# johndpope/SPEAK-hack

Measured on AMD Instinct MI355X. Metric: generator frames/sec at 256^2, batch 8/GPU, higher is better.
Workload: dtype f32; 1 GPU; StyleGAN decoder (styleganv1.StyleGenerator) 256^2 forward only, batch 8/GPU, fp32, random-init weights, synthetic [8,6144] latents, device-drawn noise; global_batch=8, resolution=256, parallelism=replicas x1 (no data-path collective), launch=hipGraph replay of the step

## Files before the change

include/spk.h:

```cpp
#ifndef SPK_H_
#define SPK_H_

#include <stddef.h>
#include <stdint.h>

#ifdef __cplusplus
extern "C" {
#endif

#define SPK_OK            0
#define SPK_EINVAL       -1
#define SPK_ELAUNCH      -2
#define SPK_EUNSUPPORTED -3

#define SPK_EPI_BIAS   1u
#define SPK_EPI_NOISE  2u
#define SPK_EPI_LRELU  4u
#define SPK_EPI_STYLE  8u
#define SPK_CONV_UPSAMPLE2X 16u
#define SPK_EPI_ACCUM  32u
#define SPK_EPI_STATS  64u
#define SPK_CONV_IN_AFFINE_RELU 128u
#define SPK_CONV_IN_BATCH_SCALE 256u
#define SPK_CONV_DGRAD_S2 1024u
#define SPK_CONV_TRANSPOSE4X4_S2 2048u
#define SPK_CONV_BF16X3 4096u
#define SPK_CONV_WINOGRAD 16384u
#define SPK_EPI_ACCUM_HALF 8192u
#define SPK_EPI_TORGB 32768u
#define SPK_EPI_RESIDUAL 65536u
#define SPK_CONV_UP_FIR1331 512u

const char* spk_version(void);
const char* spk_last_error(void);

typedef struct spk_conv2d_desc {
    const float* x;
    const float* w_packed;
    const float* bias;
    const float* noise_w;
    const float* noise;
    const float* style;
    const float* in_scale;
    const float* in_shift;
    double*      stats;
    float*       y;
    float*       y_pre;
    int32_t B, Cin, Cout;
    int32_t H, W;
    int32_t Hin, Win;
    int32_t kh, kw, stride;
    int32_t style_stride;
    uint32_t flags;
    float lrelu_slope;
    float out_scale;
    int32_t config;
    int32_t ksplit;
    void*   workspace;
    int64_t workspace_bytes;
    const float* out_scale_bc;
    float act_gain;
    int32_t groups;
    int32_t group_in_stride;
    int32_t stats_slots;
    const float* accum_half;
    const float* out_scale_dev;
    const float* rgb_w;
    const float* rgb_bias;
    float* rgb_y;
    int32_t rgb_channels;
    int32_t reserved;
    const float* residual;
} spk_conv2d_desc;

int spk_conv2d_num_configs(void);
int spk_conv2d_stats_slots(int config, int kh, int kw, int stride, int B, int Cin, int Cout, int H, int W);
int spk_conv2d_config_valid(int config, int kh, int kw, int stride);
int spk_conv2d_pick_config(int kh, int kw, int stride, int B, int Cin, int Cout, int H, int W);
int spk_conv2d_dgrad_s2_config(int B, int Cin, int Cout, int Hin, int Win);
int64_t spk_conv2d_dgrad_s2_workspace_bytes(int B, int Cin, int Cout, int Hin, int Win, int H, int W, int groups);
int spk_conv2d_config_info(int config, int* co_tile, int* ci_tile, int* pix_tile);
int64_t spk_conv2d_packed_floats(int config, int kh, int kw, int Cin, int Cout);
int64_t spk_conv2d_workspace_bytes(int config, int ksplit, int kh, int kw, int stride, int B, int Cin, int Cout,
                                   int H, int W);
int64_t spk_conv2d_workspace_bytes_grouped(int config, int ksplit, int kh, int kw, int stride, int B, int Cin, int Cout,
                                           int H, int W, int groups);
int spk_conv2d_pack_weights(const float* w, float* w_packed, int kh, int kw, int Cin, int Cout, int config,
                            int transpose_flip, void* stream);
#define SPK_PACK_LIST_MAX 8
int spk_conv2d_pack_weights_list(const float* const* ws, int n, float* w_packed, int kh, int kw, int Cin, int Cout, int config,
                                 int transpose_flip, void* stream);
int spk_conv2d_fwd(const spk_conv2d_desc* desc, void* stream);
int64_t spk_conv2d_packed_bytes_bf16x3(int Cin, int Cout);
int spk_conv2d_pack_weights_bf16x3(const float* w, void* w_packed, int Cin, int Cout, void* stream);
int spk_conv2d_pack_weights_bf16x3_tf(const float* w, void* w_packed, int Cin, int Cout, int transpose_flip, void* stream);
int spk_conv2d_bf16x3_supported(int B, int Cin, int Cout, int H, int W);
int spk_conv2d_bf16x3_fwd(const spk_conv2d_desc* desc, void* stream);

int64_t spk_conv2d_packed_bytes_wino(int Cin, int Cout);
int spk_conv2d_pack_weights_wino(const float* w, float* w_packed, int Cin, int Cout, int transpose_flip, void* stream);
#define SPK_WINO_PACK_MAX 32
int spk_conv2d_pack_weights_wino_list(const float* const* w, float* const* w_packed, const int* Cin, const int* Cout, const int* transpose_flip,
                                      int n, void* stream);
int spk_conv2d_wino_supported(int B, int Cin, int Cout, int H, int W);
int spk_conv2d_wino_up_supported(int B, int Cin, int Cout, int H, int W);
int spk_conv2d_wino_ksplit(int want, int B, int Cin, int Cout, int H, int W);
int64_t spk_conv2d_wino_workspace_bytes(int ksplit, int B, int Cin, int Cout, int H, int W);
int spk_conv2d_wino_fwd(const spk_conv2d_desc* desc, void* stream);

typedef struct spk_wgrad_desc {
    const float* g;
    const float* x;
    const float* in_scale;
    const float* in_shift;
    float*       dw;
    int32_t B, Cin, Cout, H, W, Hin, Win, kh, kw, stride;
    uint32_t flags;
    float scale;
    int32_t accumulate;
    int32_t splits;
    void*   workspace;
    int64_t workspace_bytes;
    int32_t groups;
    int32_t group_in_stride;
    int32_t fold;
    const float* g_scale;
} spk_wgrad_desc;
int64_t spk_conv2d_wgrad_workspace_bytes(int kh, int kw, int stride, int splits, int B, int Cin, int Cout, int H, int W);
int spk_conv2d_wgrad(const spk_wgrad_desc* desc, void* stream);
int spk_conv2d_wgrad_up_supported(int B, int Cin, int Cout, int H, int W);
int spk_conv2d_wgrad_mod_supported(int B, int Cin, int Cout, int H, int W, int upsample);
int spk_conv2d_wgrad_wino_supported(int B, int Cin, int Cout, int H, int W);
int spk_conv2d_wgrad_wino_splits(int splits, int B, int Cin, int Cout, int H, int W);
int64_t spk_conv2d_wgrad_wino_workspace_bytes(int splits, int B, int Cin, int Cout, int H, int W);
int spk_conv2d_wgrad_wino(const spk_wgrad_desc* desc, void* stream);
int spk_wgrad_reduce_slabs(const float* slabs, float* dw, int n_slabs, int Cout, int Cin, int taps, float scale, int accumulate, int fold,
                           void* stream);

int spk_epilogue_bwd(const float* dy, const float* a, const float* noise, const float* style, int64_t style_stride,
                     float slope, float* dt, float* sums, int B, int C, int64_t HW, void* stream);
int spk_upsample2x_bilinear_bwd(const float* dy, float* dx, int64_t planes, int Hin, int Win, void* stream);
int spk_conv1x1_small_bwd_blocks(int B, int64_t HW);
int spk_conv1x1_small_bwd(const float* x, const float* w, const float* dy, float* dx, float* partial, int B, int C, int O,
                          int64_t HW, float in_scale, void* stream);
int spk_fc_bwd(const float* dout, const float* out, const float* x, int64_t x_stride, const float* w, float* dx,
               int64_t dx_stride, float* dw, float* db, int B, int I, int O, float wmul, float bmul, float slope,
               void* stream);

int spk_fc_fwd(const float* x, int64_t x_stride, const float* w, const float* bias, float* out,
               int64_t out_stride, int B, int I, int O, float wmul, float bmul, float slope, void* stream);

#define SPK_FC_MAX_GROUPS 16
typedef struct spk_fc_group {
    const float* x;
    int64_t x_stride;
    const float* w;
    const float* bias;
    float* out;
    int64_t out_stride;
    int32_t I, O;
    float wmul, bmul, slope;
    int32_t reserved;
} spk_fc_group;
int spk_fc_grouped_fwd(const spk_fc_group* groups, int n_groups, int B, void* stream);
typedef struct spk_fc_bwd_group {
    const float* dout;
    int64_t dout_stride;
    const float* out;
    const float* x;
    int64_t x_stride;
    const float* w;
    float* dx;
    int64_t dx_stride;
    float* dw;
    float* db;
    int32_t I, O;
    float wmul, bmul, slope;
    int32_t reserved;
} spk_fc_bwd_group;
int spk_fc_grouped_bwd(const spk_fc_bwd_group* groups, int n_groups, int B, void* stream);

int spk_bias_noise_style_fwd(const float* x, int64_t x_batch_stride, const float* bias, const float* noise_w,
                             const float* noise, const float* style, int64_t style_stride, float* y, int B, int C,
                             int HW, void* stream);

int spk_conv1x1_expand_fwd(const float* x, const float* w, const float* bias, const float* scale_dev, float* y, int B, int C, int O,
                           int64_t HW, float slope, void* stream);
int spk_conv1x1_small_fwd(const float* x, const float* w, const float* bias, float* y, int B, int C, int O,
                          int64_t HW, float in_scale, void* stream);

int spk_upsample2x_bilinear_fwd(const float* x, float* y, int64_t planes, int Hin, int Win, void* stream);
int spk_upsample2x_fwd(const float* x, float* y, int64_t planes, int Hin, int Win, int zero_border, void* stream);

int spk_bn_finalize(double* stats, int stats_slots, int64_t count, const float* gamma, const float* beta, float* running_mean,
                    float* running_var, float momentum, float eps, float* scale, float* shift, float* save_mean,
                    float* save_invstd, int C, void* stream);
#define SPK_BN_LIST_MAX 64
typedef struct spk_bn_replay_item {
    const double* stats;
    float* running_mean;
    float* running_var;
    int64_t count;
    int32_t C;
    int32_t reserved;
} spk_bn_replay_item;
int spk_bn_replay_list(const spk_bn_replay_item* items_host, int n, float momentum, void* stream);
int spk_bn_add_relu_fwd(const float* a, const float* sa, const float* ba, const float* b, const float* sb,
                        const float* bb, float* y, int B, int C, int64_t HW, int relu, void* stream);
int spk_maxpool3x3s2_fwd(const float* x, const float* in_scale, const float* in_shift, float* y, int B, int C,
                         int Hin, int Win, void* stream);
int spk_bn_bwd_reduce(const float* g, const float* r, const float* mask_src, int mask_mode, const float* scale,
                      const float* shift, const float* mean, const float* invstd, float g_scale, int g_per_plane,
                      float* sums, int B, int C, int64_t HW, void* stream);
int spk_bn_bwd_apply(const float* g, const float* r, const float* mask_src, int mask_mode, const float* scale,
                     const float* shift, const float* mean, const float* invstd, const float* csum, int64_t count,
                     float g_scale, int g_per_plane, float* dr, float* dz_out, int B, int C, int64_t HW, void* stream);
int spk_bn_bwd_apply_sums(const float* g, const float* r, const float* mask_src, int mask_mode, const float* scale,
                          const float* shift, const float* mean, const float* invstd, const float* sums, float* csum_out,
                          int batch_stats, int64_t count, float g_scale, int g_per_plane, float* dr, float* dz_out, int B, int C,
                          int64_t HW, void* stream);
int spk_dilate2x(const float* x, float* y, int64_t planes, int H, int W, int Ho, int Wo, void* stream);
int spk_maxpool3x3s2_bwd(const float* x, const float* in_scale, const float* in_shift, const float* dy, float* dx, int B,
                         int C, int Hin, int Win, void* stream);
int spk_global_avgpool_fwd(const float* x, float* y, int64_t planes, int64_t HW, void* stream);

int spk_modconv_demod(const float* w, const float* s, float* d, int B, int Cin, int Cout, int taps, float scale, float eps,
                      void* stream);
int spk_modconv_epi_finish(const float* sums, const float* d, const float* bias, const float* noise_w, float gain, float* dd,
                           float* dprime, float* dbias, float* dnw, int B, int C, void* stream);
int spk_modconv_dx_finish(const float* dxt, const float* x, const float* s, float* dx, float* ds, int B, int C, int Hs, int Ws,
                          int upsample, void* stream);
int64_t spk_modconv_demod_bwd_workspace_bytes(int B, int Cin, int Cout);
int spk_modconv_demod_bwd(const float* w, const float* s, const float* d, const float* dd, float* ds, float* dw, void* workspace,
                          int64_t workspace_bytes, int B, int Cin, int Cout, int taps, float scale, void* stream);
int spk_torgb_mod_bwd_data(const float* w, const float* mod, const float* dy, float* dx, int B, int C, int O, int64_t HW,
                           float in_scale, void* stream);
#define SPK_DEMOD_MAX_GROUPS 16
typedef struct spk_demod_group {
    const float* w;
    const float* s;
    float* d;
    int32_t Cin, Cout, taps;
    float scale;
} spk_demod_group;
int spk_modconv_demod_grouped(const spk_demod_group* groups, int n_groups, int B, float eps, void* stream);
int spk_upfirdn2d_fwd(const float* x, float* y, const float* filter_host, int k, int64_t planes, int H, int W, int up, int down,
                      int pad0, int pad1, float gain, void* stream);
int spk_conv1x1_small_mod_fwd(const float* x, const float* w, const float* mod, const float* bias, float* y, int B, int C, int O,
                              int64_t HW, float in_scale, void* stream);
int spk_torgb_mod_skip_fwd(const float* x, const float* w, const float* mod, const float* bias, const float* skip, float* y, int B,
                           int C, int O, int H, int W, float in_scale, void* stream);

int spk_pixelnorm_fwd(const float* x, float* y, int B, int C, int64_t HW, float eps, int sqrt_form, void* stream);
int spk_instance_norm_affine_fwd(const float* x, float* y, const float* scale, const float* bias, int64_t sb_stride, int B, int C,
                                 int64_t HW, float eps, void* stream);
int spk_instance_norm_affine_bwd(const float* x, const float* dy, const float* scale, int64_t sb_stride, float* dx, float* dscale,
                                 float* dbias, int B, int C, int64_t HW, float eps, void* stream);
int spk_blur2d_fwd(const float* x, float* y, const float* filter_host, int k, int64_t planes, int H, int W, int stride, void* stream);
int spk_upscale2d_nearest_fwd(const float* x, float* y, int64_t planes, int H, int W, int factor, float gain, void* stream);
int spk_fade_in_tanh_fwd(const float* a, const float* b, float* y, float alpha, int64_t n, void* stream);
// ... 78 lines not shown
```

speak-hack_amd/_lib.py:

```python
from __future__ import annotations

import ctypes as C
import os
import threading

import torch

HERE = os.path.dirname(os.path.abspath(__file__))
LIB_PATH = os.path.join(HERE, "libspk_hip.so")

EPI_BIAS, EPI_NOISE, EPI_LRELU, EPI_STYLE, CONV_UPSAMPLE2X, EPI_ACCUM, EPI_STATS, CONV_IN_AFFINE_RELU = \
    1, 2, 4, 8, 16, 32, 64, 128

c_float_p = C.c_void_p


class Conv2dDesc(C.Structure):
    _fields_ = [("x", C.c_void_p), ("w_packed", C.c_void_p), ("bias", C.c_void_p), ("noise_w", C.c_void_p),
                ("noise", C.c_void_p), ("style", C.c_void_p), ("in_scale", C.c_void_p), ("in_shift", C.c_void_p),
                ("stats", C.c_void_p), ("y", C.c_void_p), ("y_pre", C.c_void_p),
                ("B", C.c_int32), ("Cin", C.c_int32), ("Cout", C.c_int32), ("H", C.c_int32), ("W", C.c_int32),
                ("Hin", C.c_int32), ("Win", C.c_int32), ("kh", C.c_int32), ("kw", C.c_int32), ("stride", C.c_int32),
                ("style_stride", C.c_int32), ("flags", C.c_uint32), ("lrelu_slope", C.c_float),
                ("out_scale", C.c_float), ("config", C.c_int32), ("ksplit", C.c_int32),
# ... 63 lines not shown


class FcGroupedArgs(C.Structure):
    _fields_ = [("groups", C.c_void_p), ("n_groups", C.c_int32), ("B", C.c_int32)]


class BiasNoiseStyleArgs(C.Structure):
    _fields_ = [("x", C.c_void_p), ("x_batch_stride", C.c_int64), ("bias", C.c_void_p), ("noise_w", C.c_void_p),
                ("noise", C.c_void_p), ("style", C.c_void_p), ("style_stride", C.c_int64), ("y", C.c_void_p),
                ("B", C.c_int32), ("C", C.c_int32), ("HW", C.c_int32), ("reserved", C.c_int32)]


class ToRGBArgs(C.Structure):
    _fields_ = [("x", C.c_void_p), ("w", C.c_void_p), ("mod", C.c_void_p), ("bias", C.c_void_p), ("skip", C.c_void_p),
                ("y", C.c_void_p), ("B", C.c_int32), ("C", C.c_int32), ("O", C.c_int32), ("H", C.c_int32), ("W", C.c_int32),
                ("in_scale", C.c_float)]


class DemodGroupedArgs(C.Structure):
    _fields_ = [("groups", C.c_void_p), ("n_groups", C.c_int32), ("B", C.c_int32), ("eps", C.c_float), ("reserved", C.c_int32)]


class Upsample2xArgs(C.Structure):
    _fields_ = [("x", C.c_void_p), ("y", C.c_void_p), ("planes", C.c_int64), ("Hin", C.c_int32), ("Win", C.c_int32),
                ("zero_border", C.c_int32), ("reserved", C.c_int32)]


class MaxPool3x3s2Args(C.Structure):
    _fields_ = [("x", C.c_void_p), ("in_scale", C.c_void_p), ("in_shift", C.c_void_p), ("y", C.c_void_p), ("B", C.c_int32),
                ("C", C.c_int32), ("Hin", C.c_int32), ("Win", C.c_int32)]


class GlobalAvgPoolArgs(C.Structure):
    _fields_ = [("x", C.c_void_p), ("y", C.c_void_p), ("planes", C.c_int64), ("HW", C.c_int64)]


class FramesToU8Args(C.Structure):
    _fields_ = [("x", C.c_void_p), ("y", C.c_void_p), ("N", C.c_int32), ("H", C.c_int32), ("W", C.c_int32), ("swap_rb", C.c_int32),
                ("lo", C.c_float), ("k", C.c_float)]


class PixelNormArgs(C.Structure):
    _fields_ = [("x", C.c_void_p), ("y", C.c_void_p), ("B", C.c_int32), ("C", C.c_int32), ("HW", C.c_int64), ("eps", C.c_float),
                ("sqrt_form", C.c_int32)]


SN_MAX_GROUPS = 24


class SnGroup(C.Structure):
    _fields_ = [("w", C.c_void_p), ("u", C.c_void_p), ("v", C.c_void_p), ("w_hat", C.c_void_p), ("sigma", C.c_void_p),
                ("dw", C.c_void_p), ("R", C.c_int32), ("C", C.c_int32), ("accumulate", C.c_int32), ("reserved", C.c_int32)]


class WgradDesc(C.Structure):
    _fields_ = [("g", C.c_void_p), ("x", C.c_void_p), ("in_scale", C.c_void_p), ("in_shift", C.c_void_p),
                ("dw", C.c_void_p),
                ("B", C.c_int32), ("Cin", C.c_int32), ("Cout", C.c_int32), ("H", C.c_int32), ("W", C.c_int32),
                ("Hin", C.c_int32), ("Win", C.c_int32), ("kh", C.c_int32), ("kw", C.c_int32), ("stride", C.c_int32),
                ("flags", C.c_uint32), ("scale", C.c_float), ("accumulate", C.c_int32), ("splits", C.c_int32),
                ("workspace", C.c_void_p), ("workspace_bytes", C.c_int64), ("groups", C.c_int32), ("group_in_stride", C.c_int32),
                ("fold", C.c_int32), ("g_scale", C.c_void_p)]


_PROTOTYPES = {
    "spk_modconv_demod": (C.c_int, [C.c_void_p, C.c_void_p, C.c_void_p, C.c_int, C.c_int, C.c_int, C.c_int, C.c_float, C.c_float,
                                    C.c_void_p]),
    "spk_modconv_demod_grouped": (C.c_int, [C.c_void_p, C.c_int, C.c_int, C.c_float, C.c_void_p]),
    "spk_upfirdn2d_fwd": (C.c_int, [C.c_void_p, C.c_void_p, C.POINTER(C.c_float), C.c_int, C.c_int64, C.c_int, C.c_int, C.c_int,
                                    C.c_int, C.c_int, C.c_int, C.c_float, C.c_void_p]),
    "spk_conv1x1_small_mod_fwd": (C.c_int, [C.c_void_p] * 5 + [C.c_int, C.c_int, C.c_int, C.c_int64, C.c_float, C.c_void_p]),
    "spk_torgb_mod_skip_fwd": (C.c_int, [C.c_void_p] * 6 + [C.c_int] * 5 + [C.c_float, C.c_void_p]),
    "spk_pixelnorm_fwd": (C.c_int, [C.c_void_p, C.c_void_p, C.c_int, C.c_int, C.c_int64, C.c_float, C.c_int, C.c_void_p]),
    "spk_instance_norm_affine_fwd": (C.c_int, [C.c_void_p, C.c_void_p, C.c_void_p, C.c_void_p, C.c_int64, C.c_int, C.c_int,
                                               C.c_int64, C.c_float, C.c_void_p]),
    "spk_instance_norm_affine_bwd": (C.c_int, [C.c_void_p, C.c_void_p, C.c_void_p, C.c_int64, C.c_void_p, C.c_void_p, C.c_void_p,
                                               C.c_int, C.c_int, C.c_int64, C.c_float, C.c_void_p]),
    "spk_blur2d_fwd": (C.c_int, [C.c_void_p, C.c_void_p, C.POINTER(C.c_float), C.c_int, C.c_int64, C.c_int, C.c_int, C.c_int,
                                 C.c_void_p]),
    "spk_upscale2d_nearest_fwd": (C.c_int, [C.c_void_p, C.c_void_p, C.c_int64, C.c_int, C.c_int, C.c_int, C.c_float, C.c_void_p]),
    "spk_fade_in_tanh_fwd": (C.c_int, [C.c_void_p, C.c_void_p, C.c_void_p, C.c_float, C.c_int64, C.c_void_p]),
    "spk_pixelnorm_bwd": (C.c_int, [C.c_void_p, C.c_void_p, C.c_void_p, C.c_int, C.c_int, C.c_int64, C.c_float, C.c_void_p]),
    "spk_blur2d_bwd": (C.c_int, [C.c_void_p, C.c_void_p, C.POINTER(C.c_float), C.c_int, C.c_int64, C.c_int, C.c_int, C.c_int,
                                 C.c_void_p]),
    "spk_avgpool2x_blend_fwd": (C.c_int, [C.c_void_p, C.c_void_p, C.c_void_p, C.c_float, C.c_float, C.c_int64, C.c_int, C.c_int,
                                          C.c_void_p]),
    "spk_avgpool2x_blend_bwd": (C.c_int, [C.c_void_p, C.c_void_p, C.c_void_p, C.c_float, C.c_float, C.c_int64, C.c_int, C.c_int,
                                          C.c_void_p]),
    "spk_minibatch_std_workspace_bytes": (C.c_int64, [C.c_int, C.c_int64]),
    "spk_minibatch_std_fwd": (C.c_int, [C.c_void_p, C.c_void_p, C.c_void_p, C.c_int, C.c_int, C.c_int64, C.c_void_p]),
    "spk_minibatch_std_bwd": (C.c_int, [C.c_void_p, C.c_void_p, C.c_void_p, C.c_void_p, C.c_int, C.c_int, C.c_int64, C.c_void_p]),
    "spk_upscale2d_nearest_bwd": (C.c_int, [C.c_void_p, C.c_void_p, C.c_int64, C.c_int, C.c_int, C.c_int, C.c_float, C.c_void_p]),
    "spk_bn_bwd_reduce": (C.c_int, [C.c_void_p, C.c_void_p, C.c_void_p, C.c_int] + [C.c_void_p] * 4 +
                          [C.c_float, C.c_int, C.c_void_p, C.c_int, C.c_int, C.c_int64, C.c_void_p]),
    "spk_bn_bwd_apply": (C.c_int, [C.c_void_p, C.c_void_p, C.c_void_p, C.c_int] + [C.c_void_p] * 5 +
                         [C.c_int64, C.c_float, C.c_int, C.c_void_p, C.c_void_p, C.c_int, C.c_int, C.c_int64, C.c_void_p]),
    "spk_bn_bwd_apply_sums": (C.c_int, [C.c_void_p, C.c_void_p, C.c_void_p, C.c_int] + [C.c_void_p] * 6 +
                              [C.c_int, C.c_int64, C.c_float, C.c_int, C.c_void_p, C.c_void_p, C.c_int, C.c_int, C.c_int64, C.c_void_p]),
    "spk_dilate2x": (C.c_int, [C.c_void_p, C.c_void_p, C.c_int64, C.c_int, C.c_int, C.c_int, C.c_int, C.c_void_p]),
    "spk_maxpool3x3s2_bwd": (C.c_int, [C.c_void_p] * 5 + [C.c_int] * 4 + [C.c_void_p]),
    "spk_conv2d_wgrad_workspace_bytes": (C.c_int64, [C.c_int] * 9),
    "spk_conv2d_wgrad": (C.c_int, [C.POINTER(WgradDesc), C.c_void_p]),
    "spk_conv2d_wgrad_up_supported": (C.c_int, [C.c_int] * 5),
    "spk_conv2d_wgrad_mod_supported": (C.c_int, [C.c_int] * 6),
    "spk_conv2d_wgrad_wino_supported": (C.c_int, [C.c_int] * 5),
    "spk_conv2d_wgrad_wino_splits": (C.c_int, [C.c_int] * 6),
    "spk_conv2d_wgrad_wino_workspace_bytes": (C.c_int64, [C.c_int] * 6),
    "spk_conv2d_wgrad_wino": (C.c_int, [C.c_void_p, C.c_void_p]),
    "spk_wgrad_reduce_slabs": (C.c_int, [C.c_void_p, C.c_void_p, C.c_int, C.c_int, C.c_int, C.c_int, C.c_float, C.c_int, C.c_int, C.c_void_p]),
    "spk_modconv_epi_finish": (C.c_int, [C.c_void_p] * 4 + [C.c_float] + [C.c_void_p] * 4 + [C.c_int, C.c_int, C.c_void_p]),
    "spk_modconv_dx_finish": (C.c_int, [C.c_void_p] * 5 + [C.c_int] * 5 + [C.c_void_p]),
    "spk_modconv_demod_bwd_workspace_bytes": (C.c_int64, [C.c_int] * 3),
    "spk_modconv_demod_bwd": (C.c_int, [C.c_void_p] * 7 + [C.c_int64] + [C.c_int] * 4 + [C.c_float, C.c_void_p]),
    "spk_torgb_mod_bwd_data": (C.c_int, [C.c_void_p] * 4 + [C.c_int, C.c_int, C.c_int, C.c_int64, C.c_float, C.c_void_p]),
    "spk_epilogue_bwd": (C.c_int, [C.c_void_p, C.c_void_p, C.c_void_p, C.c_void_p, C.c_int64, C.c_float, C.c_void_p,
                                   C.c_void_p, C.c_int, C.c_int, C.c_int64, C.c_void_p]),
    "spk_upsample2x_bilinear_bwd": (C.c_int, [C.c_void_p, C.c_void_p, C.c_int64, C.c_int, C.c_int, C.c_void_p]),
    "spk_conv1x1_small_bwd_blocks": (C.c_int, [C.c_int, C.c_int64]),
    "spk_conv1x1_small_bwd": (C.c_int, [C.c_void_p] * 5 + [C.c_int, C.c_int, C.c_int, C.c_int64, C.c_float, C.c_void_p]),
    "spk_fc_bwd": (C.c_int, [C.c_void_p, C.c_void_p, C.c_void_p, C.c_int64, C.c_void_p, C.c_void_p, C.c_int64, C.c_void_p,
                             C.c_void_p, C.c_int, C.c_int, C.c_int, C.c_float, C.c_float, C.c_float, C.c_void_p]),
    "spk_spectral_norm_workspace_bytes": (C.c_int64, [C.c_void_p, C.c_int]),
    "spk_spectral_norm_grouped": (C.c_int, [C.c_void_p, C.c_int, C.c_int, C.c_float, C.c_void_p, C.c_int64, C.c_void_p]),
    "spk_spectral_norm_bwd_grouped": (C.c_int, [C.c_void_p, C.c_int, C.c_void_p, C.c_int64, C.c_void_p]),
    "spk_launch_list": (C.c_int, [C.c_void_p, C.c_int, C.c_uint32, C.c_void_p]),
    "spk_version": (C.c_char_p, []),
    "spk_last_error": (C.c_char_p, []),
    "spk_conv2d_num_configs": (C.c_int, []),
    "spk_conv2d_config_valid": (C.c_int, [C.c_int] * 4),
    "spk_conv2d_pick_config": (C.c_int, [C.c_int] * 8),
    "spk_conv2d_dgrad_s2_config": (C.c_int, [C.c_int] * 5),
    "spk_conv2d_dgrad_s2_workspace_bytes": (C.c_int64, [C.c_int] * 8),
    "spk_conv2d_config_info": (C.c_int, [C.c_int, C.POINTER(C.c_int), C.POINTER(C.c_int), C.POINTER(C.c_int)]),
    "spk_conv2d_packed_floats": (C.c_int64, [C.c_int] * 5),
    "spk_conv2d_workspace_bytes": (C.c_int64, [C.c_int] * 10),
    "spk_conv2d_workspace_bytes_grouped": (C.c_int64, [C.c_int] * 11),
    "spk_conv2d_pack_weights": (C.c_int, [C.c_void_p, C.c_void_p, C.c_int, C.c_int, C.c_int, C.c_int, C.c_int, C.c_int,
                                          C.c_void_p]),
    "spk_conv2d_pack_weights_list": (C.c_int, [C.POINTER(C.c_void_p), C.c_int, C.c_void_p, C.c_int, C.c_int, C.c_int, C.c_int,
                                               C.c_int, C.c_int, C.c_void_p]),
    "spk_conv2d_fwd": (C.c_int, [C.POINTER(Conv2dDesc), C.c_void_p]),
    "spk_conv2d_packed_bytes_bf16x3": (C.c_int64, [C.c_int, C.c_int]),
    "spk_conv2d_pack_weights_bf16x3": (C.c_int, [C.c_void_p, C.c_void_p, C.c_int, C.c_int, C.c_void_p]),
    "spk_conv2d_pack_weights_bf16x3_tf": (C.c_int, [C.c_void_p, C.c_void_p, C.c_int, C.c_int, C.c_int, C.c_void_p]),
    "spk_conv2d_bf16x3_supported": (C.c_int, [C.c_int] * 5),
    "spk_conv2d_bf16x3_fwd": (C.c_int, [C.POINTER(Conv2dDesc), C.c_void_p]),
    "spk_conv2d_packed_bytes_wino": (C.c_int64, [C.c_int, C.c_int]),
    "spk_conv2d_pack_weights_wino": (C.c_int, [C.c_void_p, C.c_void_p, C.c_int, C.c_int, C.c_int, C.c_void_p]),
    "spk_conv2d_pack_weights_wino_list": (C.c_int, [C.c_void_p] * 5 + [C.c_int, C.c_void_p]),
    "spk_conv2d_wino_supported": (C.c_int, [C.c_int] * 5),
    "spk_conv2d_wino_up_supported": (C.c_int, [C.c_int] * 5),
    "spk_conv2d_wino_ksplit": (C.c_int, [C.c_int] * 6),
    "spk_conv2d_wino_workspace_bytes": (C.c_int64, [C.c_int] * 6),
    "spk_conv2d_wino_fwd": (C.c_int, [C.POINTER(Conv2dDesc), C.c_void_p]),
    "spk_conv2d_stats_slots": (C.c_int, [C.c_int] * 9),
    "spk_bn_finalize": (C.c_int, [C.c_void_p, C.c_int, C.c_int64, C.c_void_p, C.c_void_p, C.c_void_p, C.c_void_p, C.c_float,
                                  C.c_float, C.c_void_p, C.c_void_p, C.c_void_p, C.c_void_p, C.c_int, C.c_void_p]),
    "spk_bn_replay_list": (C.c_int, [C.c_void_p, C.c_int, C.c_float, C.c_void_p]),
    "spk_bn_add_relu_fwd": (C.c_int, [C.c_void_p] * 7 + [C.c_int, C.c_int, C.c_int64, C.c_int, C.c_void_p]),
    "spk_maxpool3x3s2_fwd": (C.c_int, [C.c_void_p] * 4 + [C.c_int] * 4 + [C.c_void_p]),
    "spk_global_avgpool_fwd": (C.c_int, [C.c_void_p, C.c_void_p, C.c_int64, C.c_int64, C.c_void_p]),
    "spk_fc_fwd": (C.c_int, [C.c_void_p, C.c_int64, C.c_void_p, C.c_void_p, C.c_void_p, C.c_int64, C.c_int, C.c_int,
                             C.c_int, C.c_float, C.c_float, C.c_float, C.c_void_p]),
    "spk_fc_grouped_fwd": (C.c_int, [C.c_void_p, C.c_int, C.c_int, C.c_void_p]),
    "spk_fc_grouped_bwd": (C.c_int, [C.c_void_p, C.c_int, C.c_int, C.c_void_p]),
    "spk_bias_noise_style_fwd": (C.c_int, [C.c_void_p, C.c_int64, C.c_void_p, C.c_void_p, C.c_void_p, C.c_void_p,
                                           C.c_int64, C.c_void_p, C.c_int, C.c_int, C.c_int, C.c_void_p]),
    "spk_conv1x1_expand_fwd": (C.c_int, [C.c_void_p] * 5 + [C.c_int, C.c_int, C.c_int, C.c_int64, C.c_float, C.c_void_p]),
    "spk_conv1x1_small_fwd": (C.c_int, [C.c_void_p, C.c_void_p, C.c_void_p, C.c_void_p, C.c_int, C.c_int, C.c_int,
                                        C.c_int64, C.c_float, C.c_void_p]),
    "spk_upsample2x_bilinear_fwd": (C.c_int, [C.c_void_p, C.c_void_p, C.c_int64, C.c_int, C.c_int, C.c_void_p]),
    "spk_plane_sums_reduce": (C.c_int, [C.c_void_p, C.c_int, C.c_int, C.c_int, C.c_int, C.c_void_p, C.c_int, C.c_void_p]),
    "spk_upsample2x_fwd": (C.c_int, [C.c_void_p, C.c_void_p, C.c_int64, C.c_int, C.c_int, C.c_int, C.c_void_p]),
    "spk_resize_table_taps": (C.c_int, [C.c_int, C.c_int]),
    "spk_resize_table": (C.c_int, [C.c_int, C.c_int, C.c_int, C.c_void_p, C.c_void_p, C.c_void_p, C.c_void_p]),
    "spk_frames_u8_to_f32": (C.c_int, [C.c_void_p, C.c_int64, C.c_int64, C.c_int, C.c_int, C.c_int, C.c_int,
                                       C.c_void_p, C.c_void_p, C.c_void_p, C.c_int, C.c_void_p, C.c_void_p, C.c_void_p, C.c_int,
                                       C.c_void_p, C.c_int, C.c_int] + [C.c_float] * 6 + [C.c_void_p]),
    "spk_frames_f32_to_u8": (C.c_int, [C.c_void_p, C.c_void_p, C.c_int, C.c_int, C.c_int, C.c_int, C.c_float, C.c_float, C.c_void_p]),
}

_lib = None
_lock = threading.Lock()


class SpkError(RuntimeError):
    pass


def exported_symbols():
    return sorted(_PROTOTYPES)


def lib():
    global _lib
    if _lib is None:
        with _lock:
            if _lib is None:
                if not os.path.exists(LIB_PATH):
                    raise SpkError(f"{LIB_PATH} is missing: build it with `python -c 'import __graft_entry__ as g; "
                                   f"g.build()'` (hipcc --offload-arch=gfx950). There is no CPU fallback.")
                h = C.CDLL(LIB_PATH)
                for name, (res, args) in _PROTOTYPES.items():
                    fn = getattr(h, name)
                    fn.restype = res
                    fn.argtypes = args
                _lib = h
    return _lib


def check(code: int, what: str):
    if code != 0:
        raise SpkError(f"{what} failed ({code}): {lib().spk_last_error().decode()}")


def stream_ptr() -> int:
    return torch.cuda.current_stream().cuda_stream


def dptr(t, name="tensor"):
    if t is None:
        return None
    if not t.is_cuda:
        raise SpkError(f"{name}: expected a HIP device tensor, got {t.device} -- speak-hack_amd has no CPU path")
    if t.dtype != torch.float32:
        raise SpkError(f"{name}: expected float32, got {t.dtype}")
    if not t.is_contiguous():
        raise SpkError(f"{name}: expected a contiguous tensor")
    return t.data_ptr()
```

speak-hack_amd/autograd.py:

```python
from __future__ import annotations

import contextlib
import functools
import weakref

import torch
from torch.utils.weak import WeakTensorKeyDictionary

from . import ops


_INPUT_GRAD_ONLY = False


@contextlib.contextmanager
def input_grad_only():
    global _INPUT_GRAD_ONLY
    prev, _INPUT_GRAD_ONLY = _INPUT_GRAD_ONLY, True
    try:
        yield
    finally:
        _INPUT_GRAD_ONLY = prev


_side_pending = set()


def _side_join(device, stream=None):
    st = ops.side_stream(device)
    if st is not None:
        (stream if stream is not None else torch.cuda.current_stream(device)).wait_stream(st)


def _wgrad_aside(dt, x, launch, extra=()):
    dev = dt.device
    side = ops.side_stream(dev)
    if side is None or torch.cuda.is_current_stream_capturing():
        return launch()
    cur = torch.cuda.current_stream(dev)
    key = (dev.index, torch._C._current_graph_task_id())
    if key not in _side_pending:
        def done(dev=dev, cur=cur, key=key):
            _side_pending.discard(key)
            _side_join(dev, cur)
        try:
            torch.autograd.Variable._execution_engine.queue_callback(done)
        except RuntimeError:
            return launch()
        _side_pending.add(key)
    side.wait_stream(cur)
    with torch.cuda.stream(side):
        ops.side_stream_delay()
        dw = launch()
    dt.record_stream(side)
    x.record_stream(side)
    for t in extra:
        t.record_stream(side)
    return dw


def _wgrad_shared(weight, a, b, make):
    task = torch._C._current_graph_task_id()
    held = getattr(weight, "_spk_dw", None)
    if held is None or held[0] != task:
        dw = _wgrad_aside(a, b, lambda: make(None, False))
        weight._spk_dw = (task, dw)
        return dw
    _wgrad_aside(a, b, lambda: make(held[1], True))
    return None


def _first_or_add(param, key, make):
    task = torch._C._current_graph_task_id()
    held = getattr(param, key, None)
    if held is None or held[0] != task:
        t = make(None)
        setattr(param, key, (task, t.detach()))
        return t
    make(held[1])
    return None


class WeightGateFn(torch.autograd.Function):

    @staticmethod
    def forward(ctx, *weights):
        ctx.dev = weights[0].device
        return tuple(w.view_as(w) for w in weights)

    @staticmethod
    @torch.autograd.function.once_differentiable
    def backward(ctx, *grads):
        _side_join(ctx.dev)
        return grads


def gate_weights(weights):
    outs = WeightGateFn.apply(*weights)
    for o, w in zip(outs, weights):
        o._spk_gate_of = w
    return outs


def _needs(ctx, grad_mode):
    return bool(grad_mode) and any(ctx.needs_input_grad)


def _epilogue_param_grads(sums, has_style, has_bias, has_noise):
    B, _, Cc = sums.shape
    dstyle = sums[:, :2].reshape(B, 2 * Cc) if has_style else None
    dbias = dnw = None
    if has_bias and has_noise:
        red = sums[:, 2:].sum(0)
        dbias, dnw = red[0], red[1]
    elif has_bias:
        dbias = sums[:, 2].sum(0)
    elif has_noise:
        dnw = sums[:, 3].sum(0)
    return dstyle, dbias, dnw


class FusedConvFn(torch.autograd.Function):

    @staticmethod
    def forward(ctx, x, weight, bias, noise_w, noise, style, upsample, slope, packed, grad_mode, w_scale=1.0):
        B, Cin, Hs, Ws = x.shape
        Cout = weight.shape[0]
        H, W = (2 * Hs, 2 * Ws) if upsample else (Hs, Ws)
        keep = _needs(ctx, grad_mode)
        a = torch.empty((B, Cout, H, W), device=x.device, dtype=torch.float32) if keep else None
        pw = getattr(weight, "_spk_gate_of", weight)
        route = ops.conv3x3_route(B, Cin, Cout, H, W)
        x2 = ops.upsample2x_bilinear(x) if upsample and route[0] == "wino" and keep else None
        y = ops.conv3x3(x if x2 is None else x2, packed.images(pw), Cout, route, upsample=upsample and x2 is None, bias=bias,
                        noise_w=noise_w, noise=noise, style=style, lrelu_slope=slope, out_pre=a, out_scale=w_scale)
        if x2 is not None and keep and ops.use_wgrad_wino(B, Cin, Cout, H, W):
            x = x2
            ctx.x_was_up = True
        if keep:
            ctx.save_for_backward(x, weight, a, noise, style)
            ctx.conf = (upsample, slope, packed, bias is not None, noise_w is not None, float(w_scale))
        return y

    @staticmethod
    @torch.autograd.function.once_differentiable
    def backward(ctx, dy):
        x, weight, a, noise, style = ctx.saved_tensors
        upsample, slope, packed, has_bias, has_noise, w_scale = ctx.conf
        x_is_up = upsample and getattr(ctx, "x_was_up", False)
        B, Cin = x.shape[:2]
        Cout, H, W = a.shape[1:]
        dt, sums = ops.epilogue_bwd(dy.contiguous(), a, noise if has_noise else None, style,
                                    slope if slope is not None else 1.0)
        dstyle, dbias, dnw = _epilogue_param_grads(sums, style is not None, has_bias, has_noise)
        dx = dw = None
        pw = getattr(weight, "_spk_gate_of", None)
        if ctx.needs_input_grad[1]:
            launch = lambda: ops.conv2d_wgrad(dt, x, Cout, Cin, 3, 1, upsample=upsample and not x_is_up, scale=w_scale)
            dw = _wgrad_aside(dt, x, launch) if pw is not None else launch()
        if pw is None:
            pw = weight
        if ctx.needs_input_grad[0]:
            dx = ops.conv3x3(dt, packed.images(pw), Cin, ops.conv3x3_route(B, Cout, Cin, H, W), transpose_flip=True, out_scale=w_scale)
            if upsample:
                dx = ops.upsample2x_bilinear_bwd(dx)
        return dx, dw, dbias, dnw, None, dstyle, None, None, None, None, None


class FCFn(torch.autograd.Function):

    @staticmethod
    def forward(ctx, x, weight, bias, wmul, bmul, slope, grad_mode):
        out = ops.fc(x, weight, bias, wmul, bmul, slope)
        if _needs(ctx, grad_mode):
            ctx.save_for_backward(x, weight, out)
            ctx.conf = (wmul, bmul, slope, bias is not None)
        return out

    @staticmethod
    def backward(ctx, dout):
        x, weight, out = ctx.saved_tensors
        wmul, bmul, slope, has_bias = ctx.conf
        if torch.is_grad_enabled():
            dx = FCDgradFn.apply(dout, out, weight, wmul, slope) if ctx.needs_input_grad[0] else None
            dw = db = None
            if not _INPUT_GRAD_ONLY and (ctx.needs_input_grad[1] or (has_bias and ctx.needs_input_grad[2])):
                with torch.no_grad():
                    _, dw, db = ops.fc_bwd(dout.detach().contiguous(), out, x, weight, wmul, bmul, slope, need_dx=False,
                                           need_dw=True, has_bias=has_bias)
            return dx, dw, db, None, None, None, None
        dx, dw, db = ops.fc_bwd(dout.contiguous(), out, x, weight, wmul, bmul, slope,
                                need_dx=ctx.needs_input_grad[0], need_dw=ctx.needs_input_grad[1] or
                                (has_bias and ctx.needs_input_grad[2]), has_bias=has_bias)
        return dx, dw, db, None, None, None, None


class FCDgradFn(torch.autograd.Function):

    @staticmethod
    def forward(ctx, dout, out, weight, wmul, slope):
        dout = dout.contiguous()
        ctx.save_for_backward(dout, out, weight)
        ctx.conf = (wmul, slope)
        dx, _, _ = ops.fc_bwd(dout, out, dout.new_empty((dout.shape[0], weight.shape[1])), weight, wmul, 0.0, slope, need_dx=True,
                              need_dw=False, has_bias=False)
        return dx

    @staticmethod
    @torch.autograd.function.once_differentiable
    def backward(ctx, g):
        dout, out, weight = ctx.saved_tensors
        wmul, slope = ctx.conf
        g = g.contiguous()
        ddout = dweight = None
        if ctx.needs_input_grad[0]:
            ddout = ops.fc(g, weight, None, wmul, 0.0, 1.0)
            if slope != 1.0:
                ddout = ddout * torch.where(out > 0, 1.0, float(slope))
        if ctx.needs_input_grad[2]:
            _, dweight, _ = ops.fc_bwd(dout, out, g, weight, wmul, 0.0, slope, need_dx=False, need_dw=True, has_bias=False)
        return ddout, None, dweight, None, None


class StyleFCGroupFn(torch.autograd.Function):

    @staticmethod
    def forward(ctx, w, confs, grad_mode, *params):
        n = len(confs)
        ws, bs = params[0::2], params[1::2]
        outs = ops.fc_grouped((w[:, j], ws[j], bs[j], confs[j][0], confs[j][1], confs[j][2]) for j in range(n))
        if _needs(ctx, grad_mode):
            ctx.save_for_backward(w, *ws, *outs)
            ctx.confs = confs
        return tuple(outs)

    @staticmethod
    @torch.autograd.function.once_differentiable
    def backward(ctx, *douts):
        confs = ctx.confs
        n = len(confs)
        saved = ctx.saved_tensors
        w, ws, outs = saved[0], saved[1:1 + n], saved[1 + n:1 + 2 * n]
        B = w.size(0)
        need_dx = ctx.needs_input_grad[0]
        live = [j for j in range(n) if douts[j] is not None]
        dwl = (torch.zeros_like(w) if (w.size(1) > n or len(live) < n) else torch.empty_like(w)) if need_dx else None
        res = ops.fc_grouped_bwd(((douts[j], outs[j], w[:, j], ws[j], dwl[:, j] if need_dx else None,
                                   ctx.needs_input_grad[3 + 2 * j] or (confs[j][3] and ctx.needs_input_grad[4 + 2 * j]),
                                   confs[j][3], confs[j][0], confs[j][1], confs[j][2]) for j in live), B) if live else []
        grads = [None] * (2 * n)
        for j, (dw, db) in zip(live, res):
            grads[2 * j], grads[2 * j + 1] = dw, db
        return (dwl, None, None, *grads)


def style_fc_group(w, linears, slope):
    confs = tuple((float(m.w_lrmul), float(m.b_lrmul), float(slope), m.bias is not None) for m in linears)
    params = [t for m in linears for t in (m.weight, m.bias)]
    return StyleFCGroupFn.apply(w, confs, torch.is_grad_enabled(), *params)


class ToRGBFn(torch.autograd.Function):

    @staticmethod
    def forward(ctx, x, weight, bias, grad_mode):
        y = ops.conv1x1_small(x, weight, bias)
        if _needs(ctx, grad_mode):
            ctx.save_for_backward(x, weight)
            ctx.has_bias = bias is not None
        return y

    @staticmethod
    @torch.autograd.function.once_differentiable
    def backward(ctx, dy):
        x, weight = ctx.saved_tensors
        dx, dw, db = ops.conv1x1_small_bwd(x, weight, dy.contiguous(), need_dx=ctx.needs_input_grad[0])
        return dx, dw, (db if ctx.has_bias else None), None


class BiasNoiseStyleFn(torch.autograd.Function):

    @staticmethod
    def forward(ctx, x, bias, noise_w, noise, style, B, grad_mode):
        y = ops.bias_noise_style(x, B, bias, noise_w, noise, style)
        if _needs(ctx, grad_mode):
# ... 579 lines not shown
```

speak-hack_amd/csrc/conv3x3_wino_f32.hip:

```cpp
#include "conv_mfma_f32.hpp"

namespace spkwino {

using spkconv::f32x16;
using spkconv::lds_f32_t;
using spkconv::static_for;
typedef float f32x2 __attribute__((ext_vector_type(2)));
typedef float f32x4 __attribute__((ext_vector_type(4)));
typedef __attribute__((address_space(3))) f32x2 lds_f32x2_t;
typedef __attribute__((address_space(3))) f32x2 __attribute__((aligned(4))) lds_f32x2u_t;

constexpr int CO_T = 64, CI_T = 8, NTILE = 64, NT = 256;
constexpr int WIDE = 0, SQUARE = 1;
constexpr int region_w(int shape) { return shape == SQUARE ? 16 : 32; }
constexpr int region_h(int shape) { return shape == SQUARE ? 16 : 8; }
constexpr int RAW_PLANE = 352, RAW_WAVE = 2 * RAW_PLANE;
constexpr int RAW_GATHERS = RAW_WAVE / 64;
constexpr int U_FLOATS = 16 * CI_T * CO_T, V_FLOATS = 16 * CI_T * NTILE, RAW_FLOATS = 4 * RAW_WAVE;
constexpr int U_OFF = 0, V_OFF = 2 * U_FLOATS, RAW_OFF = V_OFF + 2 * V_FLOATS;
constexpr int PRM_OFF = RAW_OFF + 2 * RAW_FLOATS;
constexpr int DEM_OFF = PRM_OFF + 4 * CO_T;
constexpr int RGBW_OFF = DEM_OFF + CO_T;
constexpr int LDS_FLOATS = RGBW_OFF + 3 * CO_T;
constexpr int LDS_BYTES = LDS_FLOATS * 4;
constexpr int RGB_PART_OFF = V_OFF + V_FLOATS;
static_assert(RAW_GATHERS == 11 && 34 * 10 <= RAW_PLANE && 18 * 18 <= RAW_PLANE, "geometry");
constexpr int UP_PLANE = 128, UP_GATHERS = 2 * UP_PLANE / 64;
static_assert(18 * 6 <= UP_PLANE && 10 * 10 <= UP_PLANE && 2 * UP_PLANE <= RAW_WAVE, "geometry");
constexpr int U_DMA = U_FLOATS * 4 / 1024 / 4;

struct Args {
    const float* x;
    const float* wp;
    const float* bias;
    const float* noise_w;
    const float* noise;
    const float* style;
    float* y;
    float* y_pre;
    const float* out_scale_dev;
    const float* in_scale;
    const float* out_scale_bc;
    const float* rgb_w;
    const float* rgb_bias;
    float* rgb_y;
    int B, Cin, Cout, H, W;
    int G, gin, Cx, Cy, co_tiles_g;
    int regions_x, regions_y;
    int n_chunks;
    int ksplit, cps;
    size_t slice_floats;
    int style_stride;
    unsigned flags;
    unsigned x_bytes;
    float slope, out_scale, act_gain;
};

__global__ void pack_wino_kernel(const float* __restrict__ w, float* __restrict__ out, int Cin, int Cout, int opCin, int opCout,
                                 int transpose_flip, int n_chunks, long long total) {
    const long long idx = (long long)blockIdx.x * blockDim.x + threadIdx.x;
    if (idx >= total) return;
    const int co_l = (int)(idx % CO_T);
    long long r = idx / CO_T;
    const int ci_l = (int)(r % CI_T);
    r /= CI_T;
    const int xi = (int)(r % 16);
    r /= 16;
    const int chunk = (int)(r % n_chunks), co_tile = (int)(r / n_chunks);
    const int co = co_tile * CO_T + co_l, ci = chunk * CI_T + ci_l;
    float v = 0.f;
    if (co < opCout && ci < opCin) {
        float g[3][3];
#pragma unroll
        for (int a = 0; a < 3; ++a)
#pragma unroll
            for (int b = 0; b < 3; ++b)
                g[a][b] = transpose_flip ? w[(((size_t)ci * Cin + co) * 3 + (2 - a)) * 3 + (2 - b)] : w[(((size_t)co * Cin + ci) * 3 + a) * 3 + b];
        const int i = xi >> 2, j = xi & 3;
        float t[3];
#pragma unroll
        for (int b = 0; b < 3; ++b)
            t[b] = i == 0 ? g[0][b] : (i == 3 ? g[2][b] : 0.5f * ((g[0][b] + g[2][b]) + (i == 1 ? g[1][b] : -g[1][b])));
        v = j == 0 ? t[0] : (j == 3 ? t[2] : 0.5f * ((t[0] + t[2]) + (j == 1 ? t[1] : -t[1])));
    }
    out[idx] = v;
}

struct PackWinoList {
    const float* w[SPK_WINO_PACK_MAX];
    float* out[SPK_WINO_PACK_MAX];
    int Cin[SPK_WINO_PACK_MAX], Cout[SPK_WINO_PACK_MAX], tf[SPK_WINO_PACK_MAX];
};

__global__ void pack_wino_list_kernel(const PackWinoList a) {
    const int it = blockIdx.y;
    const float* __restrict__ w = a.w[it];
    float* __restrict__ out = a.out[it];
    const int Cin = a.Cin[it], Cout = a.Cout[it], transpose_flip = a.tf[it];
    const int opCin = transpose_flip ? Cout : Cin, opCout = transpose_flip ? Cin : Cout;
    const int n_chunks = (opCin + CI_T - 1) / CI_T;
    const long long total = (long long)((opCout + CO_T - 1) / CO_T) * n_chunks * U_FLOATS;
    for (long long idx = (long long)blockIdx.x * blockDim.x + threadIdx.x; idx < total; idx += (long long)gridDim.x * blockDim.x) {
        const int co_l = (int)(idx % CO_T);
        long long r = idx / CO_T;
        const int ci_l = (int)(r % CI_T);
        r /= CI_T;
        const int xi = (int)(r % 16);
        r /= 16;
        const int chunk = (int)(r % n_chunks), co_tile = (int)(r / n_chunks);
        const int co = co_tile * CO_T + co_l, ci = chunk * CI_T + ci_l;
        float v = 0.f;
        if (co < opCout && ci < opCin) {
            float g[3][3];
#pragma unroll
            for (int p = 0; p < 3; ++p)
#pragma unroll
                for (int q = 0; q < 3; ++q)
                    g[p][q] = transpose_flip ? w[(((size_t)ci * Cin + co) * 3 + (2 - p)) * 3 + (2 - q)] : w[(((size_t)co * Cin + ci) * 3 + p) * 3 + q];
            const int i = xi >> 2, j = xi & 3;
            float t[3];
#pragma unroll
            for (int q = 0; q < 3; ++q)
                t[q] = i == 0 ? g[0][q] : (i == 3 ? g[2][q] : 0.5f * ((g[0][q] + g[2][q]) + (i == 1 ? g[1][q] : -g[1][q])));
            v = j == 0 ? t[0] : (j == 3 ? t[2] : 0.5f * ((t[0] + t[2]) + (j == 1 ? t[1] : -t[1])));
        }
        out[idx] = v;
    }
}

__device__ __forceinline__ float fadd_(float a, float b) { float r; asm("v_add_f32 %0, %1, %2" : "=v"(r) : "v"(a), "v"(b)); return r; }
__device__ __forceinline__ float fsub_(float a, float b) { float r; asm("v_sub_f32 %0, %1, %2" : "=v"(r) : "v"(a), "v"(b)); return r; }

__device__ __forceinline__ void up1d_(float a, float b, float c, float nkl, float nkr, float six, float& o0, float& o1, float& o2, float& o3) {
    float e, s, hl, hr;
    asm("v_sub_f32 %0, %1, %2" : "=v"(e) : "v"(c), "v"(a));
    asm("v_add_f32 %0, %1, %2" : "=v"(s) : "v"(a), "v"(c));
    asm("v_fma_f32 %0, %1, %2, %3" : "=v"(o1) : "v"(b), "s"(six), "v"(s));
    asm("v_fma_f32 %0, %1, %2, %3" : "=v"(hl) : "v"(b), "v"(nkl), "v"(s));
    asm("v_fma_f32 %0, %1, %2, %3" : "=v"(hr) : "v"(b), "v"(nkr), "v"(s));
    asm("v_fma_f32 %0, %1, -2.0, %2" : "=v"(o0) : "v"(e), "v"(hl));
    asm("v_fma_f32 %0, %1, -2.0, -%2" : "=v"(o3) : "v"(e), "v"(hr));
    o2 = e;
}

__device__ __forceinline__ void lds_barrier() {
    asm volatile("s_waitcnt lgkmcnt(0)\n\ts_barrier" ::: "memory");
}

template <bool MOD, int SHAPE, bool RGB = false, bool UP = false>
__global__ __launch_bounds__(NT) void wino_kernel(const Args p) {
    static_assert(!(UP && MOD), "the modulated conv keeps its x2 pass");
    constexpr int RW = region_w(SHAPE), RH = region_h(SHAPE), TXN = RW / 2, TYN = RH / 2;
    constexpr int RAW_W = UP ? RW / 2 + 2 : RW + 2, RAW_H = UP ? RH / 2 + 2 : RH + 2, RAW_USED = RAW_W * RAW_H;
    constexpr int PLANE = UP ? UP_PLANE : RAW_PLANE, NG = UP ? UP_GATHERS : RAW_GATHERS;
    extern __shared__ __attribute__((aligned(16))) float smem[];
    const int tid = threadIdx.x, lane = tid & 63;
    const int wave = __builtin_amdgcn_readfirstlane(tid >> 6);
    const int half = lane >> 5, l32 = lane & 31;
    const int wm = wave >> 1, wn = wave & 1;

    const int n_regions = p.regions_x * p.regions_y * p.B * p.ksplit;
    const int xcd = (int)blockIdx.x & 7, wk = (int)blockIdx.x >> 3, wpx = (int)gridDim.x >> 3;
    const int share_q = n_regions >> 3, share_r = n_regions & 7;
    const int reg_begin = xcd * share_q + min(xcd, share_r), reg_end = reg_begin + share_q + (xcd < share_r ? 1 : 0);
    const int grp = (int)blockIdx.y / p.co_tiles_g, co_tile = (int)blockIdx.y - grp * p.co_tiles_g, co0 = co_tile * CO_T;
    const size_t HW = (size_t)p.H * p.W;
    const int Win = UP ? p.W >> 1 : p.W;
    const size_t HWin = UP ? HW >> 2 : HW;

    const __amdgpu_buffer_rsrc_t rsrc = __builtin_amdgcn_make_buffer_rsrc(const_cast<float*>(p.x), 0, (int)p.x_bytes, 0x00020000);
    unsigned voff[NG], voff_next[NG];
    auto region_coords = [&](int item, int& b_, int& y0_, int& x0_, int& kb_) {
        const int reg = item / p.ksplit;
        kb_ = (item - reg * p.ksplit) * p.cps;
        const int rx_ = reg % p.regions_x;
        const int t_ = reg / p.regions_x;
        b_ = t_ / p.regions_y;
        y0_ = (t_ - b_ * p.regions_y) * RH;
        x0_ = rx_ * RW;
    };
    unsigned rel[NG], edge[NG];
#pragma unroll
    for (int k = 0; k < NG; ++k) {
        const int e = k * 64 + lane;
        const int j = e >= PLANE ? 1 : 0, q = e - j * PLANE;
        const int r = q / RAW_W, c = q - r * RAW_W;
        rel[k] = ((unsigned)(wave + 4 * j) * (unsigned)HWin + (unsigned)((r - 1) * Win + (c - 1))) * 4u;
        edge[k] = (r == 0 ? 1u : 0u) | (r == RAW_H - 1 ? 2u : 0u) | (c == 0 ? 4u : 0u) | (c == RAW_W - 1 ? 8u : 0u) | (q >= RAW_USED ? 16u : 0u);
    }
    auto set_voff = [&](unsigned (&vo)[NG], int b_, int y0_, int x0_) {
        const unsigned origin = (((unsigned)b_ * (unsigned)p.Cx + (unsigned)(grp * p.gin)) * (unsigned)HWin +
                                 (unsigned)(UP ? (y0_ >> 1) * Win + (x0_ >> 1) : y0_ * p.W + x0_)) * 4u;
        const unsigned at = (y0_ == 0 ? 1u : 0u) | (y0_ + RH >= p.H ? 2u : 0u) | (x0_ == 0 ? 4u : 0u) | (x0_ + RW >= p.W ? 8u : 0u) | 16u;
        if constexpr (UP) {
            const unsigned row_bytes = (unsigned)Win * 4u;
#pragma unroll
            for (int k = 0; k < NG; ++k) {
                const unsigned h = edge[k] & at;
                vo[k] = (h & 16u) ? 0x80000000u
                                  : origin + rel[k] + ((h & 1u) ? row_bytes : 0u) - ((h & 2u) ? row_bytes : 0u) + ((h & 4u) ? 4u : 0u) - ((h & 8u) ? 4u : 0u);
            }
        } else {
#pragma unroll
            for (int k = 0; k < NG; ++k) vo[k] = (edge[k] & at) ? 0x80000000u : origin + rel[k];
        }
    };
    const unsigned chunk_bytes = (unsigned)(CI_T * HWin * 4);
    const float* wsrc = p.wp + (size_t)blockIdx.y * p.n_chunks * U_FLOATS;

#define WINO_DMA_RAW(vo_in_, chunk_, slot_, k_)                                                                         \
    {                                   \
        const unsigned m0_ = (unsigned)((RAW_OFF + (slot_) * RAW_FLOATS + (k_) * 64) * 4) + raw_m0, vo_ = (vo_in_);     \
        const unsigned so_ = (unsigned)(chunk_) * chunk_bytes;                                                          \
        const __amdgpu_buffer_rsrc_t rs_ = rsrc;                                                                        \
        asm volatile("s_mov_b32 m0, %0\n\ts_nop 0\n\tbuffer_load_dword %1, %2, %3 offen lds" :: "s"(m0_), "v"(vo_), "s"(rs_), "s"(so_)); \
    }
#define WINO_DMA_U(chunk_, slot_, k_)                                                                                   \
    {                                                                                                                   \
        const unsigned m0_ = (unsigned)((U_OFF + (slot_) * U_FLOATS) * 4 + (k_) * 1024) + u_m0, vo_ = lane16;           \
        const float* sb_ = wsrc + (size_t)(chunk_) * U_FLOATS + (wave * U_DMA + (k_)) * 256;                            \
        asm volatile("s_mov_b32 m0, %0\n\ts_nop 0\n\tglobal_load_lds_dwordx4 %1, %2" :: "s"(m0_), "v"(vo_), "s"(sb_));   \
    }
    const unsigned raw_m0 = (unsigned)(wave * RAW_WAVE * 4), u_m0 = (unsigned)(wave * U_DMA * 1024), lane16 = (unsigned)lane * 16u;

    int a_base = U_OFF + half * CO_T + wm * 32 + l32;
    int b_base = V_OFF + half * NTILE + wn * 32 + l32;
    const int ty_l = lane / TXN, tx_l = lane % TXN;
    int raw_rd = (RAW_OFF + wave * RAW_WAVE + 2 * ty_l * RAW_W + 2 * tx_l) >> 1;
    int v_wr = V_OFF + wave * NTILE + lane;
    asm volatile("" : "+v"(a_base), "+v"(b_base), "+v"(raw_rd), "+v"(v_wr));
    int raw_u[2][2];
    float nk[4] = {-2.f, -2.f, -2.f, -2.f}, nkn[4] = {-2.f, -2.f, -2.f, -2.f};
    const float six = 6.f;
    auto set_nk = [&](float (&k_)[4], int y0_, int x0_) {
        k_[0] = (y0_ == 0 && ty_l == 0) ? -6.f : -2.f;
        k_[1] = (y0_ + RH >= p.H && ty_l == TYN - 1) ? -6.f : -2.f;
        k_[2] = (x0_ == 0 && tx_l == 0) ? -6.f : -2.f;
        k_[3] = (x0_ + RW >= p.W && tx_l == TXN - 1) ? -6.f : -2.f;
    };
    if constexpr (UP) {
#pragma unroll
        for (int rs = 0; rs < 2; ++rs)
#pragma unroll
            for (int j = 0; j < 2; ++j) {
                raw_u[rs][j] = RAW_OFF + wave * RAW_WAVE + ty_l * RAW_W + tx_l + rs * RAW_FLOATS + j * PLANE;
                asm volatile("" : "+v"(raw_u[rs][j]));
            }
    }

    f32x16 acc[16];
    f32x16 zero16;
#pragma unroll
    for (int r = 0; r < 16; ++r) zero16[r] = 0.f;

    float d[2][16], tq[2][16], tv[2][16];
#define WINO_T_READ(rs_, j_, r_)                                                                                        \
    {                                                                                                                   \
        const f32x2 lo_ = *((const volatile lds_f32x2_t*)0 + (raw_rd + ((rs_) * RAW_FLOATS + (j_) * RAW_PLANE + (r_) * RAW_W) / 2)); \
        const f32x2 hi_ = *((const volatile lds_f32x2_t*)0 + (raw_rd + ((rs_) * RAW_FLOATS + (j_) * RAW_PLANE + (r_) * RAW_W + 2) / 2)); \
        d[j_][4 * (r_) + 0] = lo_.x; d[j_][4 * (r_) + 1] = lo_.y; d[j_][4 * (r_) + 2] = hi_.x; d[j_][4 * (r_) + 3] = hi_.y; \
    }
#define WINO_T_ROWS(j_, c_)                                                                                             \
    {                                                                                                                   \
        tq[j_][c_] = fsub_(d[j_][c_], d[j_][8 + (c_)]); tq[j_][4 + (c_)] = fadd_(d[j_][4 + (c_)], d[j_][8 + (c_)]);     \
        tq[j_][8 + (c_)] = fsub_(d[j_][8 + (c_)], d[j_][4 + (c_)]); tq[j_][12 + (c_)] = fsub_(d[j_][4 + (c_)], d[j_][12 + (c_)]); \
    }
#define WINO_T_SCALE(j_, i_, sc_)                                                                                       \
    { tv[j_][4 * (i_)] *= (sc_); tv[j_][4 * (i_) + 1] *= (sc_); tv[j_][4 * (i_) + 2] *= (sc_); tv[j_][4 * (i_) + 3] *= (sc_); }
#define WINO_T_COLS(j_, i_)                                                                                             \
    {                                                                                                                   \
        tv[j_][4 * (i_)] = fsub_(tq[j_][4 * (i_)], tq[j_][4 * (i_) + 2]); tv[j_][4 * (i_) + 1] = fadd_(tq[j_][4 * (i_) + 1], tq[j_][4 * (i_) + 2]); \
        tv[j_][4 * (i_) + 2] = fsub_(tq[j_][4 * (i_) + 2], tq[j_][4 * (i_) + 1]); tv[j_][4 * (i_) + 3] = fsub_(tq[j_][4 * (i_) + 1], tq[j_][4 * (i_) + 3]); \
    }
#define WINO_U_READ(rs_, j_, r_)                                                                                        \
    {                                                                                                                   \
        const volatile lds_f32_t* q_ = (const volatile lds_f32_t*)0 + (raw_u[rs_][j_] + (r_) * RAW_W);                  \
        const f32x2 lo_ = *reinterpret_cast<const volatile lds_f32x2u_t*>(q_);                                          \
        d[j_][3 * (r_) + 0] = lo_.x; d[j_][3 * (r_) + 1] = lo_.y; d[j_][3 * (r_) + 2] = q_[2];                          \
    }
#define WINO_U_H(j_, r_, nk_)                                                                                           \
    up1d_(d[j_][3 * (r_)], d[j_][3 * (r_) + 1], d[j_][3 * (r_) + 2], (nk_)[2], (nk_)[3], six,                           \
          tq[j_][4 * (r_)], tq[j_][4 * (r_) + 1], tq[j_][4 * (r_) + 2], tq[j_][4 * (r_) + 3]);
#define WINO_U_V(j_, c_, nk_)                                                                                           \
    up1d_(tq[j_][c_], tq[j_][4 + (c_)], tq[j_][8 + (c_)], (nk_)[0], (nk_)[1], six,                                      \
          tv[j_][c_], tv[j_][4 + (c_)], tv[j_][8 + (c_)], tv[j_][12 + (c_)]);
#define WINO_T_WRITE(vs_, j_, xi_)                                                                                      \
    *((volatile lds_f32_t*)0 + (v_wr + ((vs_) * V_FLOATS + ((xi_) * CI_T + 4 * (j_)) * NTILE))) = tv[j_][xi_];

    if constexpr (RGB) {
        if (tid < 3 * CO_T) smem[RGBW_OFF + tid] = (tid & (CO_T - 1)) < p.Cout ? p.rgb_w[(tid >> 6) * p.Cout + (tid & (CO_T - 1))] : 0.f;
    }
    const int n = p.cps;
    int reg = reg_begin + wk;
    if (reg >= reg_end) return;
    int b, y0, x0, kb, b_cur, kb_cur;
    region_coords(reg, b, y0, x0, kb);
    b_cur = b;
    kb_cur = kb;
    set_voff(voff, b, y0, x0);
    if constexpr (UP) set_nk(nk, y0, x0);
    static_for<0, U_DMA>([&](auto k) { WINO_DMA_U(kb, 0, decltype(k)::value); });
    static_for<0, NG>([&](auto k) { WINO_DMA_RAW(voff[decltype(k)::value], kb, 0, decltype(k)::value); });
    static_for<0, NG>([&](auto k) { WINO_DMA_RAW(voff[decltype(k)::value], kb + 1, 1, decltype(k)::value); });
    __builtin_amdgcn_s_waitcnt(0x0f70);
    static_for<0, 2>([&](auto j) {
        if constexpr (UP) {
            static_for<0, 3>([&](auto r) { WINO_U_READ(0, decltype(j)::value, decltype(r)::value); });
            static_for<0, 3>([&](auto r) { WINO_U_H(decltype(j)::value, decltype(r)::value, nk); });
            static_for<0, 4>([&](auto c) { WINO_U_V(decltype(j)::value, decltype(c)::value, nk); });
        } else {
            static_for<0, 4>([&](auto r) { WINO_T_READ(0, decltype(j)::value, decltype(r)::value); });
            static_for<0, 4>([&](auto c) { WINO_T_ROWS(decltype(j)::value, decltype(c)::value); });
            static_for<0, 4>([&](auto i) { WINO_T_COLS(decltype(j)::value, decltype(i)::value); });
        }
        if constexpr (MOD) {
            const float sc0_ = p.in_scale[(size_t)b * p.Cin + kb * CI_T + wave + 4 * decltype(j)::value];
            static_for<0, 4>([&](auto i) { WINO_T_SCALE(decltype(j)::value, decltype(i)::value, sc0_); });
        }
        static_for<0, 16>([&](auto xi) { WINO_T_WRITE(0, decltype(j)::value, decltype(xi)::value); });
        __builtin_amdgcn_sched_barrier(0);
    });
    __syncthreads();

#ifndef SPK_WINO_PD
#define SPK_WINO_PD 4
#endif
    constexpr int PD = SPK_WINO_PD;
    float fa[PD + 1], fb[PD + 1];
#define WINO_FRAG(slot_, s_, reg_)                                                                                      \
    {                                                                                                                   \
        constexpr int kk_ = (s_) >> 4, xi_ = (s_) & 15;                                                                 \
        fa[reg_] = *((const volatile lds_f32_t*)0 + (a_base + ((slot_) * U_FLOATS + (xi_ * CI_T + 2 * kk_) * CO_T)));   \
        fb[reg_] = *((const volatile lds_f32_t*)0 + (b_base + ((slot_) * V_FLOATS + (xi_ * CI_T + 2 * kk_) * NTILE)));  \
    }
    auto chunk_body = [&](auto slot_c, auto first_c, const int i, const float (&nk_)[4]) __attribute__((always_inline)) {
        constexpr int S = decltype(slot_c)::value, O = 1 - S;
        constexpr bool FIRST = decltype(first_c)::value;
        const int c1 = i + 1 < n ? kb_cur + i + 1 : kb;
        const int c2 = i + 2 >= n ? kb + i + 2 - n : kb_cur + i + 2;
        float msc[2] = {1.f, 1.f};
        if constexpr (MOD) {
            const float* ms_ = p.in_scale + (size_t)(i + 1 < n ? b_cur : b) * p.Cin + c1 * CI_T + wave;
            msc[0] = ms_[0];
            msc[1] = ms_[4];
        }
        static_for<0, PD>([&](auto s) { WINO_FRAG(S, decltype(s)::value, decltype(s)::value); });
        static_for<0, 64>([&](auto s_c) {
            constexpr int s = decltype(s_c)::value;
            if constexpr (s + PD < 64) { WINO_FRAG(S, s + PD, (s + PD) % (PD + 1)); }
            if constexpr (FIRST && s < 16) acc[s & 15] = __builtin_amdgcn_mfma_f32_32x32x2f32(fa[s % (PD + 1)], fb[s % (PD + 1)], zero16, 0, 0, 0);
            else acc[s & 15] = __builtin_amdgcn_mfma_f32_32x32x2f32(fa[s % (PD + 1)], fb[s % (PD + 1)], acc[s & 15], 0, 0, 0);
            if constexpr (s < U_DMA) { WINO_DMA_U(c1, O, s); }
            else if constexpr (s < U_DMA + NG) { WINO_DMA_RAW(voff[s - U_DMA], c2, S, s - U_DMA); }
            static_for<0, 2>([&](auto j_c) {
                constexpr int j = decltype(j_c)::value, tr = 2 + 10 * j, ta = 8 + 16 * j;
                if constexpr (UP) {
                    if constexpr (s >= tr && s < tr + 3) { WINO_U_READ(O, j, s - tr); }
                    if constexpr (s >= ta && s < ta + 3) { WINO_U_H(j, s - ta, nk_); }
                    if constexpr (s >= ta + 4 && s < ta + 8) { WINO_U_V(j, s - ta - 4, nk_); }
                } else {
                if constexpr (s >= tr && s < tr + 4) { WINO_T_READ(O, j, s - tr); }
                if constexpr (s >= ta && s < ta + 4) { WINO_T_ROWS(j, s - ta); }
                if constexpr (s >= ta + 4 && s < ta + 8) { WINO_T_COLS(j, s - ta - 4); if constexpr (MOD) { WINO_T_SCALE(j, s - ta - 4, msc[j]); } }
                }
                if constexpr (s >= ta + 8 && s < ta + 16) { WINO_T_WRITE(O, j, 2 * (s - ta - 8)); WINO_T_WRITE(O, j, 2 * (s - ta - 8) + 1); }
            });
            __builtin_amdgcn_sched_barrier(0);
        });
        __builtin_amdgcn_s_waitcnt(0x0f70);
        __syncthreads();
    };
    const bool f_bias = p.flags & SPK_EPI_BIAS, f_noise = p.flags & SPK_EPI_NOISE;
    const bool f_lrelu = p.flags & SPK_EPI_LRELU, f_style = p.flags & SPK_EPI_STYLE, f_accum = p.flags & SPK_EPI_ACCUM;
    const float osc = p.out_scale_dev ? p.out_scale * *p.out_scale_dev : p.out_scale;
    const float slope_ = f_lrelu ? p.slope : 1.f, gain_ = f_lrelu ? p.act_gain : 1.f;
    const int tile = wn * 32 + l32, oy = 2 * (tile / TXN), ox = 2 * (tile % TXN);
    const int row_lane = wm * 32 + 4 * half;
    const int prm_which = tid & 3, prm_c = co0 + (tid >> 2);
    const bool prm_on = prm_c < p.Cout && (prm_which == 0 ? f_bias : (prm_which == 1 ? f_noise : f_style));
    const float* const prm_src = (prm_which == 0 ? p.bias : (prm_which == 1 ? p.noise_w : p.style + (prm_which == 3 ? p.Cout : 0))) + prm_c;
    const float prm_neutral = prm_which == 2 ? 1.f : 0.f;

    using F_ = std::false_type;
#ifdef SPK_WINO_LAB
    unsigned long long lab_t[8] = {0, 0, 0, 0, 0, 0, 0, 0};
    int lab_region = 0;
#define LAB_STAMP(k_) { if (lab_region == 1) lab_t[k_] = __builtin_readcyclecounter(); }
#else
#define LAB_STAMP(k_)
#endif
    for (;;) {
        LAB_STAMP(0)
#pragma unroll
        for (int xi = 0; xi < 16; ++xi)
#pragma unroll
            for (int r = 0; r < 16; ++r) acc[xi][r] = 0.f;
        const int cur_b = b, cur_y0 = y0, cur_x0 = x0;
        b_cur = b;
        kb_cur = kb;
        const size_t pix = (size_t)(cur_y0 + oy) * p.W + (cur_x0 + ox);
        f32x2 nz0, nz1;
        nz0.x = nz0.y = nz1.x = nz1.y = 0.f;
        if (f_noise) {
            nz0 = *reinterpret_cast<const f32x2*>(p.noise + (size_t)cur_b * HW + pix);
            nz1 = *reinterpret_cast<const f32x2*>(p.noise + (size_t)cur_b * HW + pix + p.W);
        }
        float prm = prm_neutral;
        if (prm_on) {
            const float t_ = prm_src[prm_which >= 2 ? (size_t)cur_b * p.style_stride : 0];
            prm = prm_which == 2 ? t_ + 1.f : t_;
        }
        float dem = 1.f;
        if constexpr (MOD) {
            if (p.out_scale_bc && tid < CO_T && co0 + tid < p.Cout) dem = p.out_scale_bc[(size_t)cur_b * p.Cout + co0 + tid];
        }
        const bool more = reg + wpx < reg_end;
        if (more) {
            reg += wpx;
            region_coords(reg, b, y0, x0, kb);
        }
        set_voff(voff_next, b, y0, x0);
        if constexpr (UP) {
            set_nk(nk, cur_y0, cur_x0);
            set_nk(nkn, y0, x0);
        }

        LAB_STAMP(1)
        for (int i = 0; i < n; i += 2) {
            const bool last_pair = i + 2 >= n;
#pragma unroll
            for (int k = 0; k < NG; ++k) voff[k] = last_pair ? voff_next[k] : voff[k];
            chunk_body(std::integral_constant<int, 0>{}, F_{}, i, nk);
            if constexpr (UP) {
                float nk2[4];
#pragma unroll
                for (int k = 0; k < 4; ++k) nk2[k] = last_pair ? nkn[k] : nk[k];
                chunk_body(std::integral_constant<int, 1>{}, F_{}, i + 1, nk2);
            } else {
                chunk_body(std::integral_constant<int, 1>{}, F_{}, i + 1, nk);
            }
        }

        LAB_STAMP(2)
        smem[PRM_OFF + tid] = prm;
        if constexpr (MOD) { if (tid < CO_T) smem[DEM_OFF + tid] = dem; }
        lds_barrier();
        unsigned hw_ = (unsigned)HW;
        asm volatile("" : "+s"(hw_));
        const size_t o0 = ((size_t)cur_b * p.Cy + (size_t)grp * p.Cout) * hw_ + pix + (size_t)(kb_cur / p.cps) * p.slice_floats;
        LAB_STAMP(3)
#define WINO_ACC(xi_, r_) ({ float v_; asm volatile("v_accvgpr_read_b32 %0, %1" : "=v"(v_) : "a"(acc[xi_][r_])); v_; })
        float rgb[3][4];
#pragma unroll
        for (int o = 0; o < 3; ++o)
#pragma unroll
            for (int q = 0; q < 4; ++q) rgb[o][q] = 0.f;
        static_for<0, 16>([&](auto r_c) {
            constexpr int r = decltype(r_c)::value;
            const int row = row_lane + (r & 3) + 8 * (r >> 2);
            const float4 q_ = *reinterpret_cast<const float4*>(smem + PRM_OFF + 4 * row);
            float s0[4], s1[4];
#pragma unroll
            for (int i = 0; i < 4; ++i) {
                const float m0 = WINO_ACC(4 * i, r), m1 = WINO_ACC(4 * i + 1, r), m2 = WINO_ACC(4 * i + 2, r), m3 = WINO_ACC(4 * i + 3, r);
                s0[i] = (m0 + m1) + m2;
                s1[i] = (m1 - m2) - m3;
            }
            f32x2 top, bot;
            top.x = (s0[0] + s0[1]) + s0[2]; top.y = (s1[0] + s1[1]) + s1[2];
            bot.x = (s0[1] - s0[2]) - s0[3]; bot.y = (s1[1] - s1[2]) - s1[3];
            float osc_r = osc;
            if constexpr (MOD) osc_r = osc * smem[DEM_OFF + row];
            top.x = top.x * osc_r + q_.x; top.y = top.y * osc_r + q_.x; bot.x = bot.x * osc_r + q_.x; bot.y = bot.y * osc_r + q_.x;
            top.x += q_.y * nz0.x; top.y += q_.y * nz0.y; bot.x += q_.y * nz1.x; bot.y += q_.y * nz1.y;
            top.x = (top.x > 0.f ? top.x : top.x * slope_) * gain_; top.y = (top.y > 0.f ? top.y : top.y * slope_) * gain_;
            bot.x = (bot.x > 0.f ? bot.x : bot.x * slope_) * gain_; bot.y = (bot.y > 0.f ? bot.y : bot.y * slope_) * gain_;
            const int co = co0 + row;
            if constexpr (RGB) {
                top.x = top.x * q_.z + q_.w; top.y = top.y * q_.z + q_.w; bot.x = bot.x * q_.z + q_.w; bot.y = bot.y * q_.z + q_.w;
#pragma unroll
                for (int o = 0; o < 3; ++o) {
                    const float w_ = smem[RGBW_OFF + o * CO_T + row];
                    rgb[o][0] += w_ * top.x; rgb[o][1] += w_ * top.y; rgb[o][2] += w_ * bot.x; rgb[o][3] += w_ * bot.y;
                }
                if (p.y && co < p.Cout) {
                    const size_t off = o0 + (size_t)co * hw_;
                    *reinterpret_cast<f32x2*>(p.y + off) = top;
                    *reinterpret_cast<f32x2*>(p.y + off + p.W) = bot;
                }
                __builtin_amdgcn_sched_barrier(0);
            } else if (co < p.Cout) {
                const size_t off = o0 + (size_t)co * hw_;
                if (p.y_pre) {
                    *reinterpret_cast<f32x2*>(p.y_pre + off) = top;
                    *reinterpret_cast<f32x2*>(p.y_pre + off + p.W) = bot;
                }
                top.x = top.x * q_.z + q_.w; top.y = top.y * q_.z + q_.w; bot.x = bot.x * q_.z + q_.w; bot.y = bot.y * q_.z + q_.w;
                if (f_accum) {
                    const f32x2 o_t = *reinterpret_cast<const f32x2*>(p.y + off), o_b = *reinterpret_cast<const f32x2*>(p.y + off + p.W);
                    top.x += o_t.x; top.y += o_t.y; bot.x += o_b.x; bot.y += o_b.y;
                }
#ifdef SPK_WINO_NOSTORE
                if (top.x == 12345.678f)
#endif
                {
                    *reinterpret_cast<f32x2*>(p.y + off) = top;
                    *reinterpret_cast<f32x2*>(p.y + off + p.W) = bot;
                }
            }
        });
#undef WINO_ACC
        if constexpr (RGB) {
            float* part = smem + RGB_PART_OFF + ((wm * 2 + half) * NTILE + tile) * 12;
#pragma unroll
            for (int o = 0; o < 3; ++o) *reinterpret_cast<float4*>(part + 4 * o) = make_float4(rgb[o][0], rgb[o][1], rgb[o][2], rgb[o][3]);
            lds_barrier();
            if (tid < 3 * NTILE) {
                const int o = tid >> 6, t = tid & (NTILE - 1);
                const float* ps = smem + RGB_PART_OFF + t * 12 + 4 * o;
                float4 v = *reinterpret_cast<const float4*>(ps);
#pragma unroll
                for (int g = 1; g < 4; ++g) {
                    const float4 u = *reinterpret_cast<const float4*>(ps + g * NTILE * 12);
                    v.x += u.x; v.y += u.y; v.z += u.z; v.w += u.w;
                }
                const float bo = p.rgb_bias ? p.rgb_bias[o] : 0.f;
                const size_t off = ((size_t)cur_b * 3 + o) * hw_ + (size_t)(cur_y0 + 2 * (t / TXN)) * p.W + (cur_x0 + 2 * (t % TXN));
                f32x2 a_, b_;
                a_.x = v.x + bo; a_.y = v.y + bo; b_.x = v.z + bo; b_.y = v.w + bo;
                *reinterpret_cast<f32x2*>(p.rgb_y + off) = a_;
                *reinterpret_cast<f32x2*>(p.rgb_y + off + p.W) = b_;
            }
        }
        LAB_STAMP(4)
        lds_barrier();
#ifdef SPK_WINO_LAB
        if (lab_region == 1 && blockIdx.x == 8 && blockIdx.y == 0 && tid == 0)
            for (int k = 0; k < 5; ++k) p.y[k] = (float)(long long)(lab_t[k] - lab_t[0]);
        ++lab_region;
#endif
        if (!more) break;
    }
#undef WINO_FRAG
#undef WINO_T_WRITE
#undef WINO_U_V
#undef WINO_U_H
#undef WINO_U_READ
#undef WINO_T_COLS
#undef WINO_T_SCALE
#undef WINO_T_ROWS
#undef WINO_T_READ
#undef WINO_DMA_U
#undef WINO_DMA_RAW
}

}

using namespace spkwino;

extern "C" {

int64_t spk_conv2d_packed_bytes_wino(int Cin, int Cout) {
    if (Cin <= 0 || Cout <= 0) return -1;
    return (int64_t)spk::ceil_div(Cout, CO_T) * spk::ceil_div(Cin, CI_T) * U_FLOATS * 4;
}

int spk_conv2d_pack_weights_wino(const float* w, float* w_packed, int Cin, int Cout, int transpose_flip, void* stream) {
    SPK_REQUIRE(w && w_packed && Cin > 0 && Cout > 0 && (transpose_flip == 0 || transpose_flip == 1), "pack_weights_wino: bad arguments");
    const int opCin = transpose_flip ? Cout : Cin, opCout = transpose_flip ? Cin : Cout;
    const int n_chunks = spk::ceil_div(opCin, CI_T);
    const long long total = (long long)spk::ceil_div(opCout, CO_T) * n_chunks * U_FLOATS;
    hipLaunchKernelGGL(pack_wino_kernel, dim3((unsigned)((total + 255) / 256)), dim3(256), 0, (hipStream_t)stream, w, w_packed, Cin, Cout,
                       opCin, opCout, transpose_flip, n_chunks, total);
    return spk::check_launch("pack_wino_kernel");
}

static int wino_shape(int H, int W) {
    if (H % region_h(WIDE) == 0 && W % region_w(WIDE) == 0) return WIDE;
    if (H % region_h(SQUARE) == 0 && W % region_w(SQUARE) == 0) return SQUARE;
    return -1;
}

int spk_conv2d_pack_weights_wino_list(const float* const* w, float* const* w_packed, const int* Cin, const int* Cout, const int* transpose_flip,
                                      int n, void* stream) {
    SPK_REQUIRE(w && w_packed && Cin && Cout && transpose_flip && n > 0 && n <= SPK_WINO_PACK_MAX, "pack_weights_wino_list: 1..%d items", SPK_WINO_PACK_MAX);
    PackWinoList a;
    long long most = 0;
    for (int i = 0; i < n; ++i) {
        SPK_REQUIRE(w[i] && w_packed[i] && Cin[i] > 0 && Cout[i] > 0 && (transpose_flip[i] == 0 || transpose_flip[i] == 1), "pack_weights_wino_list: item %d", i);
        a.w[i] = w[i]; a.out[i] = w_packed[i]; a.Cin[i] = Cin[i]; a.Cout[i] = Cout[i]; a.tf[i] = transpose_flip[i];
        most = std::max<long long>(most, (transpose_flip[i] ? spk_conv2d_packed_bytes_wino(Cout[i], Cin[i]) : spk_conv2d_packed_bytes_wino(Cin[i], Cout[i])) / 4);
    }
    dim3 grid((unsigned)std::min<long long>((most + 255) / 256, 2048), (unsigned)n);
    hipLaunchKernelGGL(pack_wino_list_kernel, grid, dim3(256), 0, (hipStream_t)stream, a);
    return spk::check_launch("pack_wino_list_kernel");
}

static int wino_geometry_ok(int B, int Cin, int Cout, int H, int W) {
    if (B <= 0 || Cin <= 0 || Cout <= 0 || H <= 0 || W <= 0) return 0;
    if (wino_shape(H, W) < 0) return 0;
    if (Cin % (2 * CI_T)) return 0;
    return 1;
}

int spk_conv2d_wino_supported(int B, int Cin, int Cout, int H, int W) {
    if (!wino_geometry_ok(B, Cin, Cout, H, W)) return 0;
    if ((long long)B * Cin * H * W * 4 >= (1ll << 31)) return 0;
    return 1;
}

int spk_conv2d_wino_up_supported(int B, int Cin, int Cout, int H, int W) {
    if (!wino_geometry_ok(B, Cin, Cout, H, W) || (H & 1) || (W & 1)) return 0;
    if ((long long)B * Cin * (H / 2) * (W / 2) * 4 >= (1ll << 31)) return 0;
    return 1;
}

int spk_conv2d_wino_ksplit(int want, int B, int Cin, int Cout, int H, int W) {
    if (!wino_geometry_ok(B, Cin, Cout, H, W)) return -1;
    const int shape = wino_shape(H, W), n_chunks = Cin / CI_T;
    const long long pairs = (long long)B * (H / region_h(shape)) * (W / region_w(shape)) * spk::ceil_div(Cout, CO_T);
    auto ok = [&](int ks) { return ks >= 1 && n_chunks % (2 * ks) == 0 && n_chunks / ks >= 4; };
    if (want > 0) {
        int ks = want;
        while (ks > 1 && !ok(ks)) --ks;
        return ks;
    }
    int ks = 1;
    while (pairs * ks < 192 && ok(2 * ks)) ks *= 2;
    return ks;
}

int64_t spk_conv2d_wino_workspace_bytes(int ksplit, int B, int Cin, int Cout, int H, int W) {
    const int ks = spk_conv2d_wino_ksplit(ksplit, B, Cin, Cout, H, W);
    if (ks < 0) return -1;
    return ks > 1 ? (int64_t)ks * B * Cout * H * W * 4 : 0;
}

int spk_conv2d_wino_fwd(const spk_conv2d_desc* d, void* stream) {
    SPK_REQUIRE(d && d->x && d->w_packed, "conv2d winograd: null pointer");
    SPK_REQUIRE(d->kh == 3 && d->kw == 3 && d->stride == 1, "conv2d winograd: 3x3 stride-1 kernels only");
    const int G = d->groups > 1 ? d->groups : 1;
    const bool up = d->flags & SPK_CONV_UPSAMPLE2X;
    SPK_REQUIRE(!up || (G == 1 && !(d->flags & (SPK_CONV_IN_BATCH_SCALE | SPK_CONV_UP_FIR1331))),
                "conv2d winograd: SPK_CONV_UPSAMPLE2X is the bilinear x2 of a plain launch (no IN_BATCH_SCALE, no UP_FIR1331, no groups): "
                "pass the x2 image (spk_upsample2x_fwd)");
    SPK_REQUIRE(G == 1 || !(d->flags & ~(SPK_CONV_WINOGRAD | SPK_EPI_ACCUM)), "conv2d winograd: a grouped launch takes SPK_EPI_ACCUM only (the encoders' "
                "data gradients)");
    const int gin = G > 1 ? d->group_in_stride : d->Cin, Cx = gin * (G - 1) + d->Cin, Cy = G * d->Cout;
    SPK_REQUIRE(G == 1 || gin >= d->Cin, "conv2d winograd: groups read disjoint channels");
    const unsigned epi = SPK_EPI_BIAS | SPK_EPI_NOISE | SPK_EPI_LRELU | SPK_EPI_STYLE | SPK_EPI_ACCUM;
    const unsigned allowed = SPK_CONV_WINOGRAD | epi | SPK_CONV_IN_BATCH_SCALE | SPK_EPI_TORGB | SPK_CONV_UPSAMPLE2X;
    SPK_REQUIRE(!(d->flags & ~allowed) && !d->stats && !d->accum_half,
                "conv2d winograd: plain, bilinear x2 or batch-scaled input; epilogue flags bias, noise, lrelu, style, accum, torgb");
    const bool mod = d->flags & SPK_CONV_IN_BATCH_SCALE, rgb = d->flags & SPK_EPI_TORGB;
    SPK_REQUIRE(d->y || rgb, "conv2d winograd: null pointer");
    if (rgb)
        SPK_REQUIRE(d->rgb_w && d->rgb_y && d->rgb_channels == 3 && d->Cout <= CO_T && !mod && !d->y_pre && !(d->flags & SPK_EPI_ACCUM) &&
                        (reinterpret_cast<uintptr_t>(d->rgb_y) & 7) == 0,
                    "conv2d winograd: SPK_EPI_TORGB needs rgb_w [3][Cout], rgb_y [B,3,H,W], Cout <= 64 (one channel tile), no y_pre / accumulate / modulation");
    SPK_REQUIRE(!mod || d->in_scale, "conv2d winograd: IN_BATCH_SCALE without in_scale[B,Cin]");
    SPK_REQUIRE(!d->out_scale_bc || mod, "conv2d winograd: out_scale_bc (demodulation) goes with SPK_CONV_IN_BATCH_SCALE");
    if (up)
        SPK_REQUIRE(d->H == 2 * d->Hin && d->W == 2 * d->Win && spk_conv2d_wino_up_supported(d->B, d->Cin, d->Cout, d->H, d->W),
                    "conv2d winograd: SPK_CONV_UPSAMPLE2X needs an output of twice the input size, %dx%d -> %dx%d", d->Hin, d->Win, d->H, d->W);
    else
        SPK_REQUIRE(d->H == d->Hin && d->W == d->Win, "conv2d winograd: output size must equal the input size");
    SPK_REQUIRE(wino_geometry_ok(d->B, d->Cin, d->Cout, d->H, d->W) && (long long)d->B * Cx * d->Hin * d->Win * 4 < (1ll << 31),
                "conv2d winograd: %dx%d is not a whole number of 32 x 8 or 16 x 16 regions (or the input exceeds 2 GB)", d->H, d->W);
    SPK_REQUIRE(!(d->flags & SPK_EPI_BIAS) || d->bias, "conv2d winograd: SPK_EPI_BIAS without bias");
    SPK_REQUIRE(!(d->flags & SPK_EPI_NOISE) || (d->noise && d->noise_w), "conv2d winograd: SPK_EPI_NOISE without noise");
    SPK_REQUIRE(!(d->flags & SPK_EPI_STYLE) || d->style, "conv2d winograd: SPK_EPI_STYLE without style");
    const auto aligned16 = [](const void* q) { return (reinterpret_cast<uintptr_t>(q) & 15) == 0; };
    SPK_REQUIRE(aligned16(d->w_packed) && aligned16(d->y) && aligned16(d->y_pre) && aligned16(d->noise) && (reinterpret_cast<uintptr_t>(d->x) & 3) == 0,
                "conv2d winograd: tensors must be 16-byte aligned");
    const int shape = wino_shape(d->H, d->W);
    const int ks = spk_conv2d_wino_ksplit(d->ksplit, d->B, d->Cin, Cy, d->H, d->W);
    const size_t out_floats = (size_t)d->B * Cy * d->H * d->W;
    if (ks > 1)
        SPK_REQUIRE(d->workspace && aligned16(d->workspace) && d->workspace_bytes >= (int64_t)ks * (int64_t)out_floats * 4,
                    "conv2d winograd: %d contraction slices need a workspace of %lld bytes (spk_conv2d_wino_workspace_bytes)", ks,
                    (long long)ks * (long long)out_floats * 4);
    Args a;
    a.x = d->x; a.wp = d->w_packed; a.bias = d->bias; a.noise_w = d->noise_w; a.noise = d->noise; a.style = d->style;
    a.y = d->y; a.y_pre = d->y_pre; a.out_scale_dev = d->out_scale_dev;
    a.in_scale = mod ? d->in_scale : nullptr; a.out_scale_bc = d->out_scale_bc;
    a.rgb_w = d->rgb_w; a.rgb_bias = d->rgb_bias; a.rgb_y = d->rgb_y;
    a.B = d->B; a.Cin = d->Cin; a.Cout = d->Cout; a.H = d->H; a.W = d->W;
    a.G = G; a.gin = gin; a.Cx = Cx; a.Cy = Cy; a.co_tiles_g = spk::ceil_div(d->Cout, CO_T);
    a.regions_x = d->W / region_w(shape); a.regions_y = d->H / region_h(shape);
    a.n_chunks = spk::ceil_div(d->Cin, CI_T);
    a.ksplit = ks; a.cps = a.n_chunks / ks; a.slice_floats = 0;
    a.style_stride = d->style_stride; a.flags = d->flags;
    a.x_bytes = (unsigned)((long long)d->B * Cx * d->Hin * d->Win * 4);
    const float up_scale = up ? 0.0625f : 1.f;
    a.slope = d->lrelu_slope; a.out_scale = d->out_scale * up_scale; a.act_gain = d->act_gain != 0.f ? d->act_gain : 1.f;
    SPK_REQUIRE(!rgb || ks == 1, "conv2d winograd: SPK_EPI_TORGB with a sliced contraction (%d slices): pass ksplit = 1 or run the 1x1 separately", ks);
    if (ks > 1) {
        a.y = static_cast<float*>(d->workspace); a.y_pre = nullptr; a.out_scale_dev = nullptr; a.out_scale_bc = nullptr;
        a.flags = d->flags & ~epi; a.out_scale = 1.f; a.slice_floats = out_floats;
    }
    void (*kern)(const Args) = mod ? (shape == SQUARE ? &wino_kernel<true, SQUARE> : &wino_kernel<true, WIDE>)
                               : rgb ? (shape == SQUARE ? &wino_kernel<false, SQUARE, true> : &wino_kernel<false, WIDE, true>)
                                     : (shape == SQUARE ? &wino_kernel<false, SQUARE> : &wino_kernel<false, WIDE>);
    if (up)
        kern = rgb ? (shape == SQUARE ? &wino_kernel<false, SQUARE, true, true> : &wino_kernel<false, WIDE, true, true>)
                   : (shape == SQUARE ? &wino_kernel<false, SQUARE, false, true> : &wino_kernel<false, WIDE, false, true>);
    static bool raised[10] = {false, false, false, false, false, false, false, false, false, false};
    const int which = (mod ? 2 : rgb ? 4 : 0) + (shape == SQUARE ? 1 : 0) + (up ? (rgb ? 4 : 6) : 0);
    if (!raised[which]) {
        hipError_t e = hipFuncSetAttribute(reinterpret_cast<const void*>(kern), hipFuncAttributeMaxDynamicSharedMemorySize, 160 * 1024);
        if (e != hipSuccess) return spk::fail(SPK_ELAUNCH, "hipFuncSetAttribute(LDS): %s", hipGetErrorString(e));
        raised[which] = true;
    }
    const long long n_items = (long long)a.regions_x * a.regions_y * d->B * ks;
    SPK_REQUIRE(n_items < (1ll << 31), "conv2d winograd: grid too large");
    const int co_tiles = G * spk::ceil_div(d->Cout, CO_T);
    static int n_cu = 0;
    if (n_cu == 0) {
        int dev = 0;
        hipDeviceProp_t prop;
        if (hipGetDevice(&dev) != hipSuccess || hipGetDeviceProperties(&prop, dev) != hipSuccess) return spk::fail(SPK_ELAUNCH, "conv2d winograd: no device properties");
        n_cu = prop.multiProcessorCount > 0 ? prop.multiProcessorCount : 256;
    }
    long long gx = std::max(8ll, ((long long)n_cu / co_tiles) / 8 * 8);
    static int lab_mult = -1;
    if (lab_mult < 0) { const char* e = getenv("SPK_WINO_WGS"); lab_mult = e ? atoi(e) : 1; }
    gx = lab_mult == 0 ? (n_items + 7) / 8 * 8 : gx * lab_mult;
    gx = std::min(gx, (n_items + 7) / 8 * 8);
    dim3 grid((unsigned)gx, (unsigned)co_tiles);
    hipLaunchKernelGGL(kern, grid, dim3(NT), LDS_BYTES, (hipStream_t)stream, a);
    int rc = spk::check_launch("wino_kernel");
    if (rc != SPK_OK || ks == 1) return rc;
    spkconv::ConvArgs f = {};
    f.bias = d->bias; f.noise_w = d->noise_w; f.noise = d->noise; f.style = d->style; f.out_scale_bc = d->out_scale_bc;
    f.y = d->y; f.y_pre = d->y_pre; f.B = d->B; f.Cin = d->Cin; f.Cout = d->Cout; f.Cy = Cy; f.Cx = Cx; f.G = G; f.H = d->H; f.W = d->W;
    f.style_stride = d->style_stride; f.flags = d->flags & epi; f.slope = d->lrelu_slope; f.out_scale = d->out_scale * up_scale;
    f.act_gain = a.act_gain; f.out_scale_dev = d->out_scale_dev;
    return spkconv::launch_splitk_epilogue(f, static_cast<const float*>(d->workspace), ks, (hipStream_t)stream);
}

}
```

speak-hack_amd/csrc/fc.hip:

```cpp
#include "spk_common.hpp"

namespace {

constexpr int FC_BT = 8;
constexpr int FC_WAVES = 4;

__device__ __forceinline__ void fc_dot512(const float* __restrict__ wr, const float* __restrict__ x, long long x_stride, int b0, int B,
                                          int lane, float (&acc)[FC_BT]) {
    const float4 w0 = *reinterpret_cast<const float4*>(wr + lane * 4);
    const float4 w1 = *reinterpret_cast<const float4*>(wr + 256 + lane * 4);
    float4 x0[FC_BT], x1[FC_BT];
#pragma unroll
    for (int b = 0; b < FC_BT; ++b) {
        const float* xr = x + (size_t)min(b0 + b, B - 1) * x_stride + lane * 4;
        x0[b] = *reinterpret_cast<const float4*>(xr);
        x1[b] = *reinterpret_cast<const float4*>(xr + 256);
    }
#pragma unroll
    for (int b = 0; b < FC_BT; ++b) {
        acc[b] += w0.x * x0[b].x + w0.y * x0[b].y + w0.z * x0[b].z + w0.w * x0[b].w;
        acc[b] += w1.x * x1[b].x + w1.y * x1[b].y + w1.z * x1[b].z + w1.w * x1[b].w;
    }
}

template <bool VEC>
__global__ __launch_bounds__(FC_WAVES * 64) void fc_kernel(const float* __restrict__ x, long long x_stride,
                                                          const float* __restrict__ w, const float* __restrict__ bias,
                                                          float* __restrict__ out, long long out_stride, int B, int I,
                                                          int O, float wmul, float bmul, float slope) {
    const int lane = threadIdx.x & 63;
    const int o = blockIdx.x * FC_WAVES + (threadIdx.x >> 6);
    if (o >= O) return;
    const float* wr = w + (size_t)o * I;
    const float bb = bias ? bias[o] * bmul : 0.f;
    for (int b0 = 0; b0 < B; b0 += FC_BT) {
        float acc[FC_BT];
#pragma unroll
        for (int b = 0; b < FC_BT; ++b) acc[b] = 0.f;
        if (VEC && I == 512) {
            fc_dot512(wr, x, x_stride, b0, B, lane, acc);
        } else if (VEC) {
            for (int i = lane * 4; i < I; i += 256) {
                const float4 wv = *reinterpret_cast<const float4*>(wr + i);
#pragma unroll
                for (int b = 0; b < FC_BT; ++b) {
                    if (b0 + b < B) {
                        const float4 xv = *reinterpret_cast<const float4*>(x + (size_t)(b0 + b) * x_stride + i);
                        acc[b] += wv.x * xv.x + wv.y * xv.y + wv.z * xv.z + wv.w * xv.w;
                    }
                }
            }
        } else {
            for (int i = lane; i < I; i += 64) {
                const float wv = wr[i];
#pragma unroll
                for (int b = 0; b < FC_BT; ++b)
                    if (b0 + b < B) acc[b] += wv * x[(size_t)(b0 + b) * x_stride + i];
            }
        }
#pragma unroll
        for (int b = 0; b < FC_BT; ++b) {
#pragma unroll
            for (int off = 32; off >= 1; off >>= 1) acc[b] += __shfl_xor(acc[b], off);
        }
        float v = 0.f;
#pragma unroll
        for (int b = 0; b < FC_BT; ++b)
            if (lane == b) v = acc[b];
        if (lane < FC_BT && b0 + lane < B) {
            v = v * wmul + bb;
            v = v > 0.f ? v : v * slope;
            out[(size_t)(b0 + lane) * out_stride + o] = v;
        }
    }
}


constexpr int FC_WIDE_U = 6;
__global__ __launch_bounds__(256) void fc_wide_kernel(const float* __restrict__ x, long long x_stride, const float* __restrict__ w,
                                                     const float* __restrict__ bias, float* __restrict__ out, long long out_stride,
                                                     int B, int I, int O, float wmul, float bmul, float slope) {
    __shared__ float red[4][FC_BT];
    const int tid = threadIdx.x, lane = tid & 63, wave = tid >> 6;
    const int o = blockIdx.x;
    const float* wr = w + (size_t)o * I;
    for (int b0 = 0; b0 < B; b0 += FC_BT) {
        float acc[FC_BT];
#pragma unroll
        for (int b = 0; b < FC_BT; ++b) acc[b] = 0.f;
        for (int i0 = tid * 4; i0 < I; i0 += 1024 * FC_WIDE_U) {
            float4 wv[FC_WIDE_U];
#pragma unroll
            for (int u = 0; u < FC_WIDE_U; ++u) {
                const int i = i0 + u * 1024;
                wv[u] = i < I ? *reinterpret_cast<const float4*>(wr + i) : make_float4(0.f, 0.f, 0.f, 0.f);
            }
#pragma unroll
            for (int u = 0; u < FC_WIDE_U; ++u) {
                const int i = i0 + u * 1024;
                if (i < I) {
#pragma unroll
                    for (int b = 0; b < FC_BT; ++b) {
                        if (b0 + b < B) {
                            const float4 xv = *reinterpret_cast<const float4*>(x + (size_t)(b0 + b) * x_stride + i);
                            acc[b] += wv[u].x * xv.x + wv[u].y * xv.y + wv[u].z * xv.z + wv[u].w * xv.w;
                        }
                    }
                }
            }
        }
#pragma unroll
        for (int b = 0; b < FC_BT; ++b) {
#pragma unroll
            for (int off = 32; off >= 1; off >>= 1) acc[b] += __shfl_xor(acc[b], off);
        }
        __syncthreads();
        if (lane == 0) {
#pragma unroll
            for (int b = 0; b < FC_BT; ++b) red[wave][b] = acc[b];
        }
        __syncthreads();
        if (tid < FC_BT && b0 + tid < B) {
            float v = (red[0][tid] + red[1][tid]) + (red[2][tid] + red[3][tid]);
            v = v * wmul + (bias ? bias[o] * bmul : 0.f);
            v = v > 0.f ? v : v * slope;
            out[(size_t)(b0 + tid) * out_stride + o] = v;
        }
    }
}

__global__ __launch_bounds__(256) void fc_wide4_kernel(const float* __restrict__ x, long long x_stride, const float* __restrict__ w,
                                                      const float* __restrict__ bias, float* __restrict__ out, long long out_stride,
                                                      int B, int I, int O, float wmul, float bmul, float slope) {
    __shared__ float red[4][4][FC_BT];
    const int tid = threadIdx.x, lane = tid & 63, wave = tid >> 6;
    const int o0 = blockIdx.x * 4;
    const int U = I >> 10;
    float4 wv[4][FC_WIDE_U];
#pragma unroll
    for (int r = 0; r < 4; ++r)
#pragma unroll
        for (int u = 0; u < FC_WIDE_U; ++u)
            wv[r][u] = *reinterpret_cast<const float4*>(w + (size_t)(o0 + r) * I + tid * 4 + min(u, U - 1) * 1024);
    for (int b0 = 0; b0 < B; b0 += FC_BT) {
        float acc[4][FC_BT];
#pragma unroll
        for (int r = 0; r < 4; ++r)
#pragma unroll
            for (int b = 0; b < FC_BT; ++b) acc[r][b] = 0.f;
#pragma unroll
        for (int u = 0; u < FC_WIDE_U; ++u) {
            if (u < U) {
                float4 xv[FC_BT];
#pragma unroll
                for (int b = 0; b < FC_BT; ++b)
                    xv[b] = *reinterpret_cast<const float4*>(x + (size_t)min(b0 + b, B - 1) * x_stride + tid * 4 + u * 1024);
#pragma unroll
                for (int r = 0; r < 4; ++r)
#pragma unroll
                    for (int b = 0; b < FC_BT; ++b)
                        acc[r][b] += wv[r][u].x * xv[b].x + wv[r][u].y * xv[b].y + wv[r][u].z * xv[b].z + wv[r][u].w * xv[b].w;
            }
        }
#pragma unroll
        for (int r = 0; r < 4; ++r)
#pragma unroll
            for (int b = 0; b < FC_BT; ++b) {
#pragma unroll
                for (int off = 32; off >= 1; off >>= 1) acc[r][b] += __shfl_xor(acc[r][b], off);
            }
        __syncthreads();
        if (lane == 0) {
#pragma unroll
            for (int r = 0; r < 4; ++r)
#pragma unroll
                for (int b = 0; b < FC_BT; ++b) red[wave][r][b] = acc[r][b];
        }
        __syncthreads();
        if (tid < 4 * FC_BT) {
            const int r = tid / FC_BT, b = tid % FC_BT;
            if (b0 + b < B) {
                float v = (red[0][r][b] + red[1][r][b]) + (red[2][r][b] + red[3][r][b]);
                v = v * wmul + (bias ? bias[o0 + r] * bmul : 0.f);
                v = v > 0.f ? v : v * slope;
                out[(size_t)(b0 + b) * out_stride + o0 + r] = v;
            }
        }
    }
}

struct FcGroups {
    spk_fc_group g[SPK_FC_MAX_GROUPS];
    int row_start[SPK_FC_MAX_GROUPS + 1];
    int n;
};

__global__ __launch_bounds__(FC_WAVES * 64) void fc_grouped_kernel(const FcGroups a, int B) {
    int gi = 0;
    while (gi + 1 < a.n && (int)blockIdx.x >= a.row_start[gi + 1]) ++gi;
    const spk_fc_group& g = a.g[gi];
    const int lane = threadIdx.x & 63;
    const int o = ((int)blockIdx.x - a.row_start[gi]) * FC_WAVES + (threadIdx.x >> 6);
    if (o >= g.O) return;
    const float* wr = g.w + (size_t)o * g.I;
    const float bb = g.bias ? g.bias[o] * g.bmul : 0.f;
    for (int b0 = 0; b0 < B; b0 += FC_BT) {
        float acc[FC_BT];
#pragma unroll
        for (int b = 0; b < FC_BT; ++b) acc[b] = 0.f;
        if (g.I == 512) {
            fc_dot512(wr, g.x, g.x_stride, b0, B, lane, acc);
        } else {
            for (int i = lane * 4; i < g.I; i += 256) {
                const float4 wv = *reinterpret_cast<const float4*>(wr + i);
#pragma unroll
                for (int b = 0; b < FC_BT; ++b) {
                    if (b0 + b < B) {
                        const float4 xv = *reinterpret_cast<const float4*>(g.x + (size_t)(b0 + b) * g.x_stride + i);
                        acc[b] += wv.x * xv.x + wv.y * xv.y + wv.z * xv.z + wv.w * xv.w;
                    }
                }
            }
        }
#pragma unroll
        for (int b = 0; b < FC_BT; ++b) {
#pragma unroll
            for (int off = 32; off >= 1; off >>= 1) acc[b] += __shfl_xor(acc[b], off);
        }
        float v = 0.f;
#pragma unroll
        for (int b = 0; b < FC_BT; ++b)
            if (lane == b) v = acc[b];
        if (lane < FC_BT && b0 + lane < B) {
            v = v * g.wmul + bb;
            v = v > 0.f ? v : v * g.slope;
            g.out[(size_t)(b0 + lane) * g.out_stride + o] = v;
        }
    }
}

}

extern "C" int spk_fc_fwd(const float* x, int64_t x_stride, const float* w, const float* bias, float* out,
                          int64_t out_stride, int B, int I, int O, float wmul, float bmul, float slope, void* stream) {
    SPK_REQUIRE(x && w && out, "fc: null pointer");
    SPK_REQUIRE(B > 0 && I > 0 && O > 0, "fc: bad shape B=%d I=%d O=%d", B, I, O);
    SPK_REQUIRE(x_stride >= I && out_stride >= O, "fc: row stride smaller than row");
    const bool vec = (I % 4 == 0) && (x_stride % 4 == 0) && ((uintptr_t)x % 16 == 0) && ((uintptr_t)w % 16 == 0);
    if (vec && I >= 2048 && I % 1024 == 0 && I <= 1024 * FC_WIDE_U && O % 4 == 0) {
        hipLaunchKernelGGL(fc_wide4_kernel, dim3((unsigned)(O / 4)), dim3(256), 0, (hipStream_t)stream, x, (long long)x_stride, w, bias, out,
                           (long long)out_stride, B, I, O, wmul, bmul, slope);
        return spk::check_launch("fc_wide4_kernel");
    }
    if (vec && I >= 2048) {
        hipLaunchKernelGGL(fc_wide_kernel, dim3((unsigned)O), dim3(256), 0, (hipStream_t)stream, x, (long long)x_stride, w, bias, out,
                           (long long)out_stride, B, I, O, wmul, bmul, slope);
        return spk::check_launch("fc_wide_kernel");
    }
    dim3 grid((unsigned)spk::ceil_div(O, FC_WAVES)), block(FC_WAVES * 64);
    if (vec)
        hipLaunchKernelGGL(fc_kernel<true>, grid, block, 0, (hipStream_t)stream, x, (long long)x_stride, w, bias, out,
                           (long long)out_stride, B, I, O, wmul, bmul, slope);
    else
        hipLaunchKernelGGL(fc_kernel<false>, grid, block, 0, (hipStream_t)stream, x, (long long)x_stride, w, bias, out,
                           (long long)out_stride, B, I, O, wmul, bmul, slope);
    return spk::check_launch("fc_kernel");
}

extern "C" int spk_fc_grouped_fwd(const spk_fc_group* groups, int n_groups, int B, void* stream) {
    SPK_REQUIRE(groups && n_groups > 0 && n_groups <= SPK_FC_MAX_GROUPS && B > 0, "fc_grouped: bad arguments (1..%d groups)",
                SPK_FC_MAX_GROUPS);
    FcGroups a;
    a.n = n_groups;
    a.row_start[0] = 0;
    for (int i = 0; i < n_groups; ++i) {
        const spk_fc_group& g = groups[i];
        SPK_REQUIRE(g.x && g.w && g.out && g.I > 0 && g.O > 0 && g.x_stride >= g.I && g.out_stride >= g.O, "fc_grouped: group %d: bad shape", i);
        SPK_REQUIRE(g.I % 4 == 0 && g.x_stride % 4 == 0 && (uintptr_t)g.x % 16 == 0 && (uintptr_t)g.w % 16 == 0,
                    "fc_grouped: group %d: rows must be 16-byte aligned multiples of 4 floats", i);
        a.g[i] = g;
        a.row_start[i + 1] = a.row_start[i] + spk::ceil_div(g.O, FC_WAVES);
    }
    hipLaunchKernelGGL(fc_grouped_kernel, dim3((unsigned)a.row_start[n_groups]), dim3(FC_WAVES * 64), 0, (hipStream_t)stream, a, B);
    return spk::check_launch("fc_grouped_kernel");
}
```

speak-hack_amd/ops.py:

```python
from __future__ import annotations

import ctypes as C
import contextlib
import weakref

import os

import torch

from . import _lib as L



def _launch_conv2d(desc):
    L.check(L.lib().spk_conv2d_fwd(C.byref(desc), L.stream_ptr()), "spk_conv2d_fwd")


def _run_conv2d(desc, ws_bytes, device):
    if ws_bytes > 0:
        ws = _workspace(device, ws_bytes)
        desc.workspace, desc.workspace_bytes = ws.data_ptr(), ws.numel() * 4
    _launch_conv2d(desc)


_KIND_FLAGS = L.CONV_WINOGRAD | L.CONV_BF16X3 | L.CONV_TRANSPOSE4X4_S2 | L.CONV_DGRAD_S2


def conv_desc(x, w_packed, Cout, k=3, stride=1, *, flags=0, out=None, hw=None, bias=None, noise_w=None, noise=None, style=None,
              style_stride=None, upsample=False, up_fir=False, lrelu_slope=None, out_scale=1.0, in_affine=None, batch_scale=None,
              demod=None, act_gain=1.0, stats=None, out_pre=None, accumulate=False, accum_half=None, out_scale_dev=None, config=-1,
              ksplit=0, groups=1, shared_input=False, rgb_w=None, rgb_bias=None, rgb_out=None, residual=None):
    B, Cin, Hs, Ws = x.shape
    G = int(groups)
    if G > 1 and not shared_input:
        if Cin % G:
            raise L.SpkError(f"conv2d: {Cin} input channels do not split into {G} groups")
        Cin //= G
    if hw is not None:
        H, W = hw
    elif upsample:
        H, W = 2 * Hs, 2 * Ws
    else:
        H, W = conv_out_size(Hs, k, stride), conv_out_size(Ws, k, stride)
    if noise is not None and (noise_w is None or noise.numel() != B * H * W):
        raise L.SpkError(f"conv2d: noise must be [B,1,H,W]={B, 1, H, W}, got {tuple(noise.shape)}")
    if accum_half is not None and (tuple(accum_half.shape) != (B, G * Cout, (H + 1) // 2, (W + 1) // 2) or not accum_half.is_contiguous()):
        raise L.SpkError(f"conv2d: accum_half must be a contiguous {(B, G * Cout, (H + 1) // 2, (W + 1) // 2)} tensor")
    if batch_scale is not None and (tuple(batch_scale.shape) != (B, Cin) or in_affine is not None):
        raise L.SpkError("conv2d: batch_scale must be [B,Cin] and excludes in_affine")
    if demod is not None and (batch_scale is None or tuple(demod.shape) != (B, Cout)):
        raise L.SpkError("conv2d: demod must be [B,Cout] and goes with batch_scale")
    if residual is not None and (tuple(residual.shape) != (B, G * Cout, H, W) or k != 1 or stride != 1):
        raise L.SpkError(f"conv2d: residual must be {(B, G * Cout, H, W)} and goes with a stride-1 1x1 conv")
    slots = 0
    if stats is not None:
        slots = stats.numel() // (2 * G * Cout)
        if (stats.dtype != torch.float64 or not stats.is_cuda or not stats.is_contiguous() or slots < 1
                or stats.numel() != slots * 2 * G * Cout):
            raise L.SpkError("conv2d: stats must be a contiguous float64 HIP tensor of slots*2*groups*Cout elements (see stats_slots)")
    if style is not None and style_stride is None:
        style_stride = style.stride(0) if style.dim() == 2 else 2 * Cout
    flags |= ((L.EPI_BIAS if bias is not None else 0) | (L.EPI_NOISE if noise is not None else 0)
              | (L.EPI_LRELU if lrelu_slope is not None else 0) | (L.EPI_STYLE if style is not None else 0)
              | (L.CONV_UPSAMPLE2X | (L.CONV_UP_FIR1331 if up_fir else 0) if upsample else 0) | (L.EPI_ACCUM if accumulate else 0)
              | (L.CONV_IN_AFFINE_RELU if in_affine is not None else 0) | (L.EPI_ACCUM_HALF if accum_half is not None else 0)
              | (L.CONV_IN_BATCH_SCALE if batch_scale is not None else 0) | (L.EPI_STATS if stats is not None else 0)
              | (L.EPI_TORGB if rgb_w is not None else 0) | (L.EPI_RESIDUAL if residual is not None else 0))
    kind = flags & _KIND_FLAGS
    if kind & (L.CONV_BF16X3 | L.CONV_TRANSPOSE4X4_S2):
        ksplit = 1
    if kind == 0 and config < 0:
        config = _modulated_config(conv2d_pick_config(k, stride, B, Cin, Cout, H, W), batch_scale is not None)
    if kind == 0:
        ws_bytes = L.lib().spk_conv2d_workspace_bytes_grouped(int(config), int(ksplit), k, k, stride, B, Cin, Cout, H, W, G)
        if ws_bytes < 0:
            raise L.SpkError(f"conv2d: config {config} cannot host k={k} s={stride} shape {(B, Cin, Cout, H, W)}")
    elif kind == L.CONV_WINOGRAD:
        ws_bytes = L.lib().spk_conv2d_wino_workspace_bytes(int(ksplit), B, Cin, G * Cout, H, W)
    elif kind == L.CONV_DGRAD_S2:
        ws_bytes = L.lib().spk_conv2d_dgrad_s2_workspace_bytes(B, Cin, Cout, Hs, Ws, H, W, G)
    else:
        ws_bytes = 0
    d = L.Conv2dDesc(x=L.dptr(x, "x"), w_packed=w_packed.data_ptr() if w_packed.dtype == torch.uint8 else L.dptr(w_packed, "w_packed"),
                     bias=L.dptr(bias, "bias"), noise_w=L.dptr(noise_w, "noise_w") if noise is not None else None,
                     noise=L.dptr(noise, "noise"), style=_style_ptr(style),
                     in_scale=L.dptr(in_affine[0], "in_scale") if in_affine is not None else L.dptr(batch_scale, "batch_scale"),
                     in_shift=L.dptr(in_affine[1], "in_shift") if in_affine is not None else None,
                     out_scale_bc=L.dptr(demod, "demod"), act_gain=float(act_gain),
                     stats=stats.data_ptr() if stats is not None else None, y=L.dptr(out, "out"), y_pre=L.dptr(out_pre, "out_pre"),
                     B=B, Cin=Cin, Cout=Cout, H=H, W=W, Hin=Hs, Win=Ws, kh=k, kw=k, stride=stride, style_stride=int(style_stride or 0),
                     flags=flags, lrelu_slope=float(lrelu_slope if lrelu_slope is not None else 1.0), out_scale=float(out_scale),
                     config=int(config), ksplit=int(ksplit), workspace=None, workspace_bytes=0, groups=G,
                     group_in_stride=0 if (shared_input or G == 1) else Cin, stats_slots=slots,
                     accum_half=L.dptr(accum_half, "accum_half"), out_scale_dev=L.dptr(out_scale_dev, "out_scale_dev"),
                     rgb_w=L.dptr(rgb_w, "rgb weight"), rgb_bias=L.dptr(rgb_bias, "rgb bias"), rgb_y=L.dptr(rgb_out, "rgb_out"),
                     rgb_channels=3 if rgb_w is not None else 0, residual=L.dptr(residual, "residual"))
    return d, ws_bytes


class PackedConvWeight:

    def __init__(self):
        self._cache = {}

    def get(self, weight, key, transpose_flip=False) -> torch.Tensor:
        ws = list(weight) if isinstance(weight, (list, tuple)) else [weight]
        hit, out = self._lookup(ws, (key, transpose_flip))
        if hit is None:
            ds = [w.detach() for w in ws]
            if len(ds) == 1:
                hit = pack_image(ds[0], key, transpose_flip, out=out)
            elif key == "wino":
                hit = out if out is not None else empty_image("wino", *_op_channels(ds[0], transpose_flip), ds[0].device, len(ds))
                pack_conv_weights_wino_into(ds, list(hit.view(len(ds), -1)), transpose_flip)
            else:
                hit = pack_conv_weights_list(ds, key, transpose_flip, out=out)
            self._put(ws, (key, transpose_flip), hit)
        return hit

    def get_wino(self, weight, transpose_flip: bool = False) -> torch.Tensor:
        return self.get(weight, "wino", bool(transpose_flip))

    def images(self, weight):
        return lambda key, transpose_flip: (self.get(weight, key, transpose_flip), None)

    @staticmethod
    def _stamp(weights):
        return [(w.data_ptr(), w._version, w.shape) for w in weights]

    def _lookup(self, weights, cache_key):
        hit = self._cache.get(cache_key)
        if hit is None:
            return None, None
        stamp, image, refs = hit
        now = self._stamp(weights)
        if now == stamp and all(r() is w for r, w in zip(refs, weights)):
            return image, None
        same_size = [s[2] for s in now] == [s[2] for s in stamp] and image.device == weights[0].device
        return None, image if same_size else None

    def _put(self, weights, cache_key, image):
        self._cache[cache_key] = (self._stamp(weights), image, [weakref.ref(w) for w in weights])

    def clear(self):
        self._cache.clear()


def conv2d_pick_config(k, stride, B, Cin, Cout, H, W) -> int:
    cfg = L.lib().spk_conv2d_pick_config(k, k, stride, B, Cin, Cout, H, W)
    if cfg < 0:
        raise L.SpkError(f"spk_conv2d_pick_config: {L.lib().spk_last_error().decode()}")
    return cfg


def conv2d_config_fits(config: int, k, stride, B, Cin, Cout, H, W) -> bool:
    return L.lib().spk_conv2d_workspace_bytes(int(config), 1, k, k, stride, B, Cin, Cout, H, W) >= 0


def conv2d_config_info(config: int):
    co, ci, px = C.c_int(), C.c_int(), C.c_int()
    L.check(L.lib().spk_conv2d_config_info(config, C.byref(co), C.byref(ci), C.byref(px)), "spk_conv2d_config_info")
    return co.value, ci.value, px.value


def pack_conv_weight(weight: torch.Tensor, config: int, transpose_flip=False, out=None) -> torch.Tensor:
    return pack_conv_weights_list([weight], config, transpose_flip, out=out)


PACK_LIST_MAX = 8


def pack_conv_weights_list(weights, config: int, transpose_flip=False, out=None) -> torch.Tensor:
    w0 = weights[0]
    tf = int(transpose_flip)
    if tf == 3:
        Cin, Cout, kh, kw = w0.shape
        n1 = L.lib().spk_conv2d_packed_floats(config, 2, 2, Cin, 4 * Cout)
    else:
        Cout, Cin, kh, kw = w0.shape
        if tf == 2:
            n1 = L.lib().spk_conv2d_packed_floats(config, 2, 2, Cout, 4 * Cin)
        else:
            n1 = L.lib().spk_conv2d_packed_floats(config, kh, kw, Cout if tf else Cin, Cin if tf else Cout)
    if n1 <= 0:
        raise L.SpkError("spk_conv2d_packed_floats: bad arguments")
    if out is None:
        out = torch.empty(n1 * len(weights), device=w0.device, dtype=torch.float32)
    elif out.numel() != n1 * len(weights) or not out.is_contiguous() or out.device != w0.device:
        raise L.SpkError(f"pack_conv_weights_list: out must be a contiguous buffer of {n1 * len(weights)} floats on {w0.device}")
    ws = [w.contiguous() for w in weights]
    if any(w.shape != w0.shape or w.device != w0.device for w in ws):
        raise L.SpkError("pack_conv_weights_list: the weights must share shape and device")
    for i in range(0, len(ws), PACK_LIST_MAX):
        part = ws[i:i + PACK_LIST_MAX]
        arr = (C.c_void_p * len(part))(*[L.dptr(w, "weight") for w in part])
        L.check(L.lib().spk_conv2d_pack_weights_list(arr, len(part), L.dptr(out) + 4 * n1 * i, kh, kw, Cin, Cout, config, tf,
                                                     L.stream_ptr()),
                "spk_conv2d_pack_weights_list")
    return out


_workspaces = {}
_retired = []


def _workspace(device, nbytes: int):
    key = (device, torch.cuda.current_stream(device).cuda_stream)
    ws = _workspaces.get(key)
    if ws is None or ws.numel() * 4 < nbytes:
        fresh = torch.empty((max(nbytes, 1 << 20) + 3) // 4, device=device, dtype=torch.float32)
        if torch.cuda.is_current_stream_capturing():
            return fresh
        if ws is not None:
            _retired.append(ws)
        ws = _workspaces[key] = fresh
    return ws


_side_streams = {}


def side_stream(device):
    if os.environ.get("SPK_WGRAD_STREAM", "1") == "0":
        return None
    key = torch.device(device).index if torch.device(device).index is not None else torch.cuda.current_device()
    st = _side_streams.get(key)
    if st is None:
        st = _side_streams[key] = torch.cuda.Stream(device, priority=int(os.environ.get("SPK_WGRAD_STREAM_PRIORITY", "0")))
    return st


def side_stream_delay():
    n = int(os.environ.get("SPK_WGRAD_STREAM_DELAY", "0"))
    if n > 0:
        torch.cuda._sleep(n)


def conv_out_size(n, k, stride):
    return (n + 2 * ((k - 1) // 2) - k) // stride + 1


def conv2d_fused(x, w_packed, Cout: int, k: int = 3, stride: int = 1, *, bias=None, noise_w=None, noise=None,
                 style=None, style_stride=None, upsample=False, lrelu_slope=None, out_scale=1.0, in_affine=None,
                 stats=None, config=-1, ksplit=0, out=None, accumulate=False, out_pre=None, batch_scale=None, demod=None,
                 act_gain=1.0, up_fir=False, groups=1, shared_input=False, accum_half=None, out_scale_dev=None):
    B, _, Hs, Ws = x.shape
    H, W = (2 * Hs, 2 * Ws) if upsample else (conv_out_size(Hs, k, stride), conv_out_size(Ws, k, stride))
    if out is None:
        out = torch.empty((B, int(groups) * Cout, H, W), device=x.device, dtype=torch.float32)
    d, ws_bytes = conv_desc(x, w_packed, Cout, k, stride, out=out, bias=bias, noise_w=noise_w, noise=noise, style=style,
                            style_stride=style_stride, upsample=upsample, up_fir=up_fir, lrelu_slope=lrelu_slope, out_scale=out_scale,
                            in_affine=in_affine, stats=stats, config=config, ksplit=ksplit, accumulate=accumulate, out_pre=out_pre,
                            batch_scale=batch_scale, demod=demod, act_gain=act_gain, groups=groups, shared_input=shared_input,
                            accum_half=accum_half, out_scale_dev=out_scale_dev)
    _run_conv2d(d, ws_bytes, x.device)
    return out


def bf16x3_supported(B, Cin, Cout, H, W) -> bool:
    return bool(L.lib().spk_conv2d_bf16x3_supported(B, Cin, Cout, H, W))


def pack_conv_weight_bf16x3(weight: torch.Tensor, out=None, transpose_flip=False) -> torch.Tensor:
    Cout, Cin, kh, kw = weight.shape
    if (kh, kw) != (3, 3):
        raise L.SpkError("pack_conv_weight_bf16x3: 3x3 kernels only")
    n = L.lib().spk_conv2d_packed_bytes_bf16x3(Cout, Cin) if transpose_flip else L.lib().spk_conv2d_packed_bytes_bf16x3(Cin, Cout)
    if out is None:
        out = torch.empty(n, device=weight.device, dtype=torch.uint8)
    elif out.numel() * out.element_size() != n or not out.is_contiguous():
        raise L.SpkError(f"pack_conv_weight_bf16x3: out must hold {n} bytes")
    L.check(L.lib().spk_conv2d_pack_weights_bf16x3_tf(L.dptr(weight.contiguous(), "weight"), out.data_ptr(), Cin, Cout,
                                                      1 if transpose_flip else 0, L.stream_ptr()),
            "spk_conv2d_pack_weights_bf16x3_tf")
    return out


TRAIN_CONV_PRECISION = "f32"
BF16X3_MIN_PIXELS = 2048


@contextlib.contextmanager
def train_conv_precision(precision: str):
    global TRAIN_CONV_PRECISION
    if precision not in ("f32", "bf16x3"):
        raise ValueError("precision must be 'f32' or 'bf16x3'")
    prev, TRAIN_CONV_PRECISION = TRAIN_CONV_PRECISION, precision
    try:
        yield
    finally:
        TRAIN_CONV_PRECISION = prev


def conv3x3_bf16x3(x, w_packed, Cout, *, bias=None, noise_w=None, noise=None, style=None, upsample=False, up_fir=False,
                   lrelu_slope=None, out_scale=1.0, batch_scale=None, demod=None, act_gain=1.0, out=None, out_pre=None):
    B, _, Hs, Ws = x.shape
    if out is None:
        out = torch.empty((B, Cout, 2 * Hs, 2 * Ws) if upsample else (B, Cout, Hs, Ws), device=x.device, dtype=torch.float32)
    d, _ = conv_desc(x, w_packed, Cout, flags=L.CONV_BF16X3, out=out, bias=bias, noise_w=noise_w, noise=noise, style=style,
                     upsample=upsample, up_fir=up_fir, lrelu_slope=lrelu_slope, out_scale=out_scale, batch_scale=batch_scale,
                     demod=demod, act_gain=act_gain, out_pre=out_pre)
    _launch_conv2d(d)
    return out


CONV3X3_ALGO = os.environ.get("SPK_CONV3X3_ALGO", "auto")
WINO_MIN_WORKGROUPS = 192
WINO_FUSE_X2 = os.environ.get("SPK_WINO_FUSE_X2", "1") != "0"


@contextlib.contextmanager
def conv3x3_algo(algo: str):
    global CONV3X3_ALGO
    if algo not in ("auto", "direct"):
        raise ValueError("conv3x3 algo must be 'auto' or 'direct'")
    prev, CONV3X3_ALGO = CONV3X3_ALGO, algo
    try:
        yield
    finally:
        CONV3X3_ALGO = prev


def use_wino(B, Cin, Cout, H, W, groups=1) -> bool:
    if CONV3X3_ALGO != "auto" or not wino_supported(B, Cin, Cout, H, W):
        return False
    rw, rh = (32, 8) if (W % 32 == 0 and H % 8 == 0) else (16, 16)
    tiles = groups * ((Cout + 63) // 64)
    return B * (H // rh) * (W // rw) * tiles * wino_ksplit(B, Cin, groups * Cout, H, W) >= WINO_MIN_WORKGROUPS


def wino_ksplit(B, Cin, Cout, H, W, want=0) -> int:
    return int(L.lib().spk_conv2d_wino_ksplit(int(want), B, Cin, Cout, H, W))


def wino_supported(B, Cin, Cout, H, W) -> bool:
    return bool(L.lib().spk_conv2d_wino_supported(B, Cin, Cout, H, W))


def wino_fuse_x2(B, Cin, Cout, H, W, up_fir=False, modulated=False) -> bool:
    return bool(WINO_FUSE_X2 and not up_fir and not modulated and L.lib().spk_conv2d_wino_up_supported(B, Cin, Cout, H, W))


def pack_conv_weight_wino(weight: torch.Tensor, out=None, transpose_flip=False) -> torch.Tensor:
    Cout, Cin, kh, kw = weight.shape
    if (kh, kw) != (3, 3):
        raise L.SpkError("pack_conv_weight_wino: 3x3 kernels only")
    n = (L.lib().spk_conv2d_packed_bytes_wino(Cout, Cin) if transpose_flip else L.lib().spk_conv2d_packed_bytes_wino(Cin, Cout)) // 4
    if out is None:
        out = torch.empty(n, device=weight.device, dtype=torch.float32)
    elif out.numel() != n or out.dtype != torch.float32 or not out.is_contiguous():
        raise L.SpkError(f"pack_conv_weight_wino: out must hold {n} floats")
    L.check(L.lib().spk_conv2d_pack_weights_wino(L.dptr(weight.contiguous(), "weight"), L.dptr(out), Cin, Cout,
                                                 1 if transpose_flip else 0, L.stream_ptr()), "spk_conv2d_pack_weights_wino")
    return out


WINO_PACK_MAX = 32


def pack_conv_weights_wino_into(weights, outs, transpose_flip=False):
    tfs = list(transpose_flip) if isinstance(transpose_flip, (list, tuple)) else [transpose_flip] * len(weights)
    for i in range(0, len(weights), WINO_PACK_MAX):
        ws, os_, tf = weights[i:i + WINO_PACK_MAX], outs[i:i + WINO_PACK_MAX], tfs[i:i + WINO_PACK_MAX]
        n = len(ws)
        keep = [w.contiguous() for w in ws]
        L.check(L.lib().spk_conv2d_pack_weights_wino_list((C.c_void_p * n)(*[L.dptr(w, "weight") for w in keep]),
                                                          (C.c_void_p * n)(*[o.data_ptr() for o in os_]),
                                                          (C.c_int * n)(*[w.shape[1] for w in ws]), (C.c_int * n)(*[w.shape[0] for w in ws]),
                                                          (C.c_int * n)(*[1 if t else 0 for t in tf]), n, L.stream_ptr()),
                "spk_conv2d_pack_weights_wino_list")


def prepack_wino(items):
    todo = []
    for pk, w, tf in items:
        hit, out = pk._lookup([w], ("wino", bool(tf)))
        if hit is None:
            todo.append((pk, w, bool(tf), out if out is not None else empty_image("wino", *_op_channels(w, tf), w.device)))
    if todo:
        pack_conv_weights_wino_into([w.detach() for _, w, _, _ in todo], [out for *_, out in todo], [tf for _, _, tf, _ in todo])
    for pk, w, tf, out in todo:
        pk._put([w], ("wino", tf), out)


def upsample2x(x, zero_border=False):
    B, Cc, H, W = x.shape
    y = torch.empty((B, Cc, 2 * H, 2 * W), device=x.device, dtype=torch.float32)
    L.check(L.lib().spk_upsample2x_fwd(L.dptr(x.contiguous(), "x"), L.dptr(y), B * Cc, H, W, 1 if zero_border else 0, L.stream_ptr()),
            "spk_upsample2x_fwd")
    return y


def conv3x3_wino(x, w_packed, Cout, *, bias=None, noise_w=None, noise=None, style=None, style_stride=None, lrelu_slope=None,
                 out_scale=1.0, act_gain=1.0, out=None, out_pre=None, accumulate=False, out_scale_dev=None, batch_scale=None, demod=None,
                 ksplit=0, rgb=None, rgb_out=None, store_out=True, groups=1, upsample=False):
    B, _, H, W = x.shape
    if upsample:
        H, W = 2 * H, 2 * W
    G = int(groups)
    if G > 1 and any(t is not None for t in (bias, noise, style, out_pre, batch_scale, demod, rgb, lrelu_slope)):
        raise L.SpkError("conv3x3_wino: a grouped launch is plain (accumulate allowed)")
    rgb_w2d, rgb_bias = None, None
    if rgb is not None:
        if Cout > 64 or out_pre is not None or accumulate or batch_scale is not None or tuple(rgb[0].shape[:2]) != (3, Cout):
            raise L.SpkError("conv3x3_wino: a fused toRGB needs Cout <= 64, weight [3,Cout,1,1], no out_pre / accumulate / modulation")
        if rgb_out is None:
            rgb_out = torch.empty((B, 3, H, W), device=x.device, dtype=torch.float32)
        ksplit = 1
        rgb_w2d, rgb_bias = rgb[0].detach().reshape(3, Cout).contiguous(), rgb[1]
    if out is None and (rgb is None or store_out):
        out = torch.empty((B, G * Cout, H, W), device=x.device, dtype=torch.float32)
    d, ws_bytes = conv_desc(x, w_packed, Cout, flags=L.CONV_WINOGRAD, out=out, bias=bias, noise_w=noise_w, noise=noise, style=style,
                            style_stride=style_stride, lrelu_slope=lrelu_slope, out_scale=out_scale, act_gain=act_gain, out_pre=out_pre,
                            accumulate=accumulate, out_scale_dev=out_scale_dev, batch_scale=batch_scale, demod=demod, ksplit=ksplit,
                            groups=G, rgb_w=rgb_w2d, rgb_bias=rgb_bias, rgb_out=rgb_out if rgb is not None else None, upsample=upsample)
    _run_conv2d(d, ws_bytes, x.device)
    return (out, rgb_out) if rgb is not None else out


def _bf16x3_route(precision, B, Cin, Cout, H, W) -> bool:
    return (precision == "bf16x3" and B * H * W >= BF16X3_MIN_PIXELS and bf16x3_supported(B, Cin, Cout, H, W)
            and not (H * W <= 256 and use_wino(B, Cin, Cout, H, W)))


def train_bf16x3(B, Cin, Cout, H, W) -> bool:
    return _bf16x3_route(TRAIN_CONV_PRECISION, B, Cin, Cout, H, W)


def _modulated_config(config, modulated):
    return config + 4 if modulated and config < 4 else config


def conv3x3_route(B, Cin, Cout, H, W, *, precision=None, groups=1, modulated=False, up_w=None, wino_ok=True):
    if _bf16x3_route(TRAIN_CONV_PRECISION if precision is None else precision, B, Cin, Cout, H, W):
        return "bf16x3", -1
    if wino_ok and (up_w is None or up_w % 4 == 0) and use_wino(B, Cin, Cout, H, W, groups):
        return "wino", -1
    return "direct", _modulated_config(conv2d_pick_config(3, 1, B, Cin, Cout, H, W), modulated)


def conv3x3(x, images, Cout, route, *, transpose_flip=False, upsample=False, up_fir=False, **epilogue):
    kind, config = route
    image, scale_dev = images(config if kind == "direct" else kind, transpose_flip)
    if scale_dev is not None:
        epilogue["out_scale_dev"] = scale_dev
    if kind == "bf16x3":
        return conv3x3_bf16x3(x, image, Cout, upsample=upsample, up_fir=up_fir, **epilogue)
    if kind == "wino":
        if upsample and wino_fuse_x2(x.shape[0], x.shape[1], Cout, 2 * x.shape[2], 2 * x.shape[3], up_fir,
                                     modulated=epilogue.get("batch_scale") is not None):
            return conv3x3_wino(x, image, Cout, upsample=True, **epilogue)
        if upsample:
            x = upsample2x(x, zero_border=True) if up_fir else upsample2x_bilinear(x)
        return conv3x3_wino(x, image, Cout, **epilogue)
    return conv2d_fused(x, image, Cout, 3, 1, config=config, upsample=upsample, up_fir=up_fir, **epilogue)


def pack_image(weight: torch.Tensor, key, transpose_flip=False, out=None) -> torch.Tensor:
    if key == "wino":
        return pack_conv_weight_wino(weight, out=out, transpose_flip=transpose_flip)
    if key == "bf16x3":
        return pack_conv_weight_bf16x3(weight, out=out, transpose_flip=transpose_flip)
    return pack_conv_weight(weight, key, transpose_flip, out=out)


def empty_image(key, Cin, Cout, device, count=1) -> torch.Tensor:
    if key == "bf16x3":
        return torch.empty(count * L.lib().spk_conv2d_packed_bytes_bf16x3(Cin, Cout), device=device, dtype=torch.uint8)
    n = L.lib().spk_conv2d_packed_bytes_wino(Cin, Cout) // 4 if key == "wino" else L.lib().spk_conv2d_packed_floats(key, 3, 3, Cin, Cout)
    return torch.empty(count * n, device=device, dtype=torch.float32)


def _op_channels(weight, transpose_flip):
    Cout, Cin = weight.shape[:2]
    return (Cout, Cin) if transpose_flip else (Cin, Cout)


def conv3x3_pick_config(B, Cin, Cout, H, W) -> int:
    return conv2d_pick_config(3, 1, B, Cin, Cout, H, W)


def conv3x3_config_fits(config, B, Cin, Cout, H, W) -> bool:
    return conv2d_config_fits(config, 3, 1, B, Cin, Cout, H, W)


conv3x3_config_info = conv2d_config_info
pack_conv3x3_weight = pack_conv_weight


def conv3x3_fused(x, w_packed, Cout, **kw):
    return conv2d_fused(x, w_packed, Cout, 3, 1, **kw)


def _style_ptr(style):
    if style is None:
        return None
    if not style.is_cuda or style.dtype != torch.float32 or style.stride(-1) != 1:
        raise L.SpkError("style: expected a float32 HIP tensor with unit inner stride")
    return style.data_ptr()


def fc(x, weight, bias=None, wmul=1.0, bmul=1.0, slope=1.0, out=None):
    if x.dim() != 2 or x.stride(1) != 1:
        raise L.SpkError("fc: x must be 2-D with unit inner stride")
    B, I = x.shape
    O = weight.shape[0]
    if weight.shape[1] != I:
        raise L.SpkError(f"fc: weight {tuple(weight.shape)} does not match input width {I}")
    if out is None:
        out = torch.empty((B, O), device=x.device, dtype=torch.float32)
    if out.stride(1) != 1:
        raise L.SpkError("fc: out must have unit inner stride")
    if not x.is_cuda or x.dtype != torch.float32:
        raise L.SpkError(f"fc: expected a float32 HIP tensor, got {x.dtype} on {x.device} (no CPU path)")
    L.check(L.lib().spk_fc_fwd(x.data_ptr(), x.stride(0), L.dptr(weight, "weight"), L.dptr(bias, "bias"),
                               out.data_ptr(), out.stride(0), B, I, O, float(wmul), float(bmul), float(slope),
                               L.stream_ptr()), "spk_fc_fwd")
    return out


def fc_grouped(items):
    items = list(items)
    outs, groups = [], (L.FcGroup * len(items))()
    B = items[0][0].shape[0]
    for g, (x, weight, bias, wmul, bmul, slope) in zip(groups, items):
        if x.dim() != 2 or x.stride(1) != 1 or x.shape[0] != B or not x.is_cuda or x.dtype != torch.float32:
            raise L.SpkError("fc_grouped: every x must be a float32 HIP [B,I] view with unit inner stride")
        O, I = weight.shape
        out = torch.empty((B, O), device=x.device, dtype=torch.float32)
        outs.append(out)
        g.x, g.x_stride, g.w, g.bias = x.data_ptr(), x.stride(0), L.dptr(weight, "weight"), L.dptr(bias, "bias")
        g.out, g.out_stride, g.I, g.O = out.data_ptr(), O, I, O
        g.wmul, g.bmul, g.slope = float(wmul), float(bmul), float(slope)
    L.check(L.lib().spk_fc_grouped_fwd(C.cast(groups, C.c_void_p), len(items), B, L.stream_ptr()), "spk_fc_grouped_fwd")
    return outs


def fc_grouped_bwd(items, B):
    items = list(items)
    groups, res, keep = (L.FcBwdGroup * len(items))(), [], []
    for g, (dout, out, x, weight, dx, need_dw, has_bias, wmul, bmul, slope) in zip(groups, items):
        O, I = weight.shape
        if dout.dim() != 2 or dout.stride(1) != 1 or dout.stride(0) < O:
            dout = dout.contiguous()
        keep.append(dout)
        if x.stride(1) != 1 or (dx is not None and dx.stride(1) != 1):
            raise L.SpkError("fc_grouped_bwd: x / dx must have unit inner stride")
        dw = torch.empty((O, I), device=weight.device, dtype=torch.float32) if need_dw else None
        db = torch.empty(O, device=weight.device, dtype=torch.float32) if (need_dw and has_bias) else None
        res.append((dw, db))
        g.dout, g.dout_stride, g.out, g.x, g.x_stride = dout.data_ptr(), dout.stride(0), L.dptr(out, "out"), x.data_ptr(), x.stride(0)
        g.w, g.dx, g.dx_stride = L.dptr(weight, "weight"), (dx.data_ptr() if dx is not None else None), (dx.stride(0) if dx is not None else 0)
        g.dw, g.db, g.I, g.O = L.dptr(dw), L.dptr(db), I, O
        g.wmul, g.bmul, g.slope = float(wmul), float(bmul), float(slope)
    L.check(L.lib().spk_fc_grouped_bwd(C.cast(groups, C.c_void_p), len(items), B, L.stream_ptr()), "spk_fc_grouped_bwd")
    return res


def bias_noise_style(x, B: int, bias=None, noise_w=None, noise=None, style=None):
    xb, Cc, H, W = x.shape
    if xb not in (1, B):
        raise L.SpkError(f"bias_noise_style: batch {xb} does not broadcast to {B}")
    if noise is not None and noise.numel() != B * H * W:
        raise L.SpkError(f"bias_noise_style: noise must be [B,1,H,W], got {tuple(noise.shape)}")
    out = torch.empty((B, Cc, H, W), device=x.device, dtype=torch.float32)
    L.check(L.lib().spk_bias_noise_style_fwd(L.dptr(x, "x"), 0 if xb == 1 and B > 1 else Cc * H * W,
                                             L.dptr(bias, "bias"),
                                             L.dptr(noise_w, "noise_w") if noise is not None else None,
                                             L.dptr(noise, "noise"), _style_ptr(style),
                                             style.stride(0) if style is not None else 0, L.dptr(out), B, Cc, H * W,
                                             L.stream_ptr()), "spk_bias_noise_style_fwd")
    return out


def const_prologue(const_in, bias, noise_w, noise, style, B: int):
    return bias_noise_style(const_in, B, bias, noise_w, noise, style)


def conv1x1_small(x, weight, bias=None, in_scale=1.0):
    B, Cc, H, W = x.shape
    O = weight.shape[0]
    out = torch.empty((B, O, H, W), device=x.device, dtype=torch.float32)
    L.check(L.lib().spk_conv1x1_small_fwd(L.dptr(x, "x"), L.dptr(weight.reshape(O, Cc), "weight"), L.dptr(bias, "bias"),
                                          L.dptr(out), B, Cc, O, H * W, float(in_scale), L.stream_ptr()),
            "spk_conv1x1_small_fwd")
    return out


# ... 710 lines not shown
```

speak-hack_amd/plan.py:

```python
from __future__ import annotations

import ctypes as C
import os

import torch

from . import _lib as L
from . import ops

LRELU = 0.2
FUSE_TORGB = os.environ.get("SPK_FUSE_TORGB", "1") != "0"
MAX_PLANS = 4


def _sig(params):
    return tuple((p.data_ptr(), p._version) for p in params)


class LaunchPlan:
    def __init__(self, device):
        self.device = device
        self.ops = []
        self.keep = []
        self._array = None
        self._refreshers = []
        self._params = []
        self._where = []
        self._stamp = None
        self.captured = False
        self.ws = None
        self._ws_bytes = 0
        self._up_scratch, self._up_users = None, []

    def buf(self, *shape):
        t = torch.empty(shape, device=self.device, dtype=torch.float32)
        self.keep.append(t)
        return t

    def add(self, kind, desc):
        self.ops.append((kind, desc))
        return desc

    def track(self, *params):
        self._params.extend(params)

    def conv(self, x, weight, Cout, *, bias=None, noise_w=None, noise=None, style=None, upsample=False, up_fir=False, slope=None,
             out, out_scale=1.0, batch_scale=None, demod=None, act_gain=1.0, precision="f32"):
        B, Cin, Hs, Ws = x.shape
        H, W = (2 * Hs, 2 * Ws) if upsample else (Hs, Ws)
        kind, cfg = ops.conv3x3_route(B, Cin, Cout, H, W, precision=precision, modulated=batch_scale is not None,
                                      up_w=Ws if upsample else None)
        up_op = None
        if kind == "wino" and upsample and ops.wino_fuse_x2(B, Cin, Cout, H, W, up_fir, modulated=batch_scale is not None):
            pass
        elif kind == "wino" and upsample:
            need = B * Cin * H * W
            if self._up_scratch is None or self._up_scratch.numel() < need:
                self._up_scratch = self.buf(need)
                for a_, n_ in self._up_users:
                    a_.y = self._up_scratch.data_ptr()
                    n_.x = self._up_scratch.data_ptr()
            xu = self._up_scratch[:need].view(B, Cin, H, W)
            up_op = self.add(L.OP_UPSAMPLE2X, L.Upsample2xArgs(x=x.data_ptr(), y=xu.data_ptr(), planes=B * Cin, Hin=Hs, Win=Ws,
                                                               zero_border=1 if up_fir else 0))
            x, upsample = xu, False
        key = cfg if kind == "direct" else kind
        packed = ops.empty_image(key, Cin, Cout, self.device)
        self.keep.append(packed)
        self._refreshers.append(lambda w=weight, p=packed, k=key: ops.pack_image(w.detach(), k, out=p))
        self.track(weight)
        d, ws_bytes = ops.conv_desc(x, packed, Cout, flags={"wino": L.CONV_WINOGRAD, "bf16x3": L.CONV_BF16X3}.get(kind, 0), out=out,
                                    bias=bias, noise_w=noise_w, noise=noise, style=style, upsample=upsample, up_fir=up_fir,
                                    lrelu_slope=slope, out_scale=out_scale, batch_scale=batch_scale, demod=demod, act_gain=act_gain,
                                    config=cfg)
        self._ws_bytes = max(self._ws_bytes, ws_bytes)
        if up_op is not None:
            self._up_users.append((up_op, d))
        return self.add(L.OP_CONV2D, d)

    def fc(self, x, lin_weight, lin_bias, wmul, bmul, slope, out):
        self.track(lin_weight, *([lin_bias] if lin_bias is not None else []))
        O, I = lin_weight.shape
        return self.add(L.OP_FC, L.FcArgs(x=x.data_ptr(), x_stride=x.stride(0), w=L.dptr(lin_weight, "weight"),
                                           bias=L.dptr(lin_bias, "bias"), out=out.data_ptr(), out_stride=out.stride(0),
                                           B=x.shape[0], I=I, O=O, wmul=float(wmul), bmul=float(bmul), slope=float(slope)))

    def fc_grouped(self, items, B):
        arr = (L.FcGroup * len(items))()
        for g, (x, xs, weight, bias, wmul, bmul, slope, out) in zip(arr, items):
            self.track(weight, *([bias] if bias is not None else []))
            O, I = weight.shape
            g.x, g.x_stride, g.w, g.bias = (x.data_ptr() if x is not None else None), xs, L.dptr(weight, "weight"), L.dptr(bias, "bias")
            g.out, g.out_stride, g.I, g.O = out.data_ptr(), out.stride(0), I, O
            g.wmul, g.bmul, g.slope = float(wmul), float(bmul), float(slope)
        self.keep.append(arr)
        self.add(L.OP_FC_GROUPED, L.FcGroupedArgs(groups=C.addressof(arr), n_groups=len(items), B=B))
        return arr

    def finish(self, *owners):
        loc = {}
        for owner in owners:
            for m in owner.modules():
                for n, q in m._parameters.items():
                    if q is not None:
                        loc.setdefault(id(q), (m, n))
        self._where = [loc.get(id(q)) for q in self._params]
        if self._ws_bytes:
            self.ws = self.buf((self._ws_bytes + 3) // 4)
            for kind, d in self.ops:
                if kind == L.OP_CONV2D:
                    d.workspace, d.workspace_bytes = self.ws.data_ptr(), self.ws.numel() * 4
        self._array = (L.Op * len(self.ops))()
        for slot, (kind, d) in zip(self._array, self.ops):
            slot.kind, slot.desc = kind, C.addressof(d)
        self.refresh(force=True)

    def refresh(self, force=False):
        stamp = _sig(self._params)
        if force or stamp != self._stamp:
            with torch.no_grad():
                for f in self._refreshers:
                    f()
            self._stamp = stamp

    def valid_for(self):
        if self._stamp is None:
            return False
        for a, q, w in zip(self._stamp, self._params, self._where):
            if a[0] != q.data_ptr() or (w is not None and w[0]._parameters.get(w[1]) is not q):
                return False
        return True

    def launch(self, kind_mask=L.ALL_OPS):
        L.check(L.lib().spk_launch_list(C.addressof(self._array), len(self.ops), int(kind_mask) & 0xFFFFFFFF, L.stream_ptr()),
                "spk_launch_list")


class DecoderPlan(LaunchPlan):

    def __init__(self, synthesis, B, device, generator=None, precision="f32", output="f32", value_range=(-1, 1), swap_rb=False):
        super().__init__(device)
        if output not in ("f32", "uint8"):
            raise ValueError(f"DecoderPlan: output must be 'f32' or 'uint8', got {output!r}")
        s = self.synthesis = synthesis
        self.precision = precision
        self.output = output
        self.B, self.with_mapping = B, generator is not None
        mods = [s.style_mod] + [m for layer in s.layers for m in (layer.style_mod1, layer.style_mod2)]
        if len(mods) > L.FC_MAX_GROUPS:
            raise L.SpkError("DecoderPlan: too many style affines for one grouped launch")
        psi = [1.0] * len(mods)
        self.feat_fc = None
        if generator is not None:
            w_in = None
            for i, fc in enumerate(generator.mapping):
                out = self.buf(B, fc.weight.shape[0])
                if i == 0:
                    self.feat_fc = self.add(L.OP_FC, L.FcArgs(x=None, x_stride=fc.weight.shape[1], w=L.dptr(fc.weight, "weight"),
                                                              bias=L.dptr(fc.bias, "bias"), out=out.data_ptr(), out_stride=out.stride(0),
                                                              B=B, I=fc.weight.shape[1], O=fc.weight.shape[0], wmul=float(fc.w_lrmul),
                                                              bmul=float(fc.b_lrmul), slope=LRELU))
                    self.track(fc.weight, fc.bias)
                else:
                    self.fc(w_in, fc.weight, fc.bias, fc.w_lrmul, fc.b_lrmul, LRELU, out)
                w_in = out
            self.w512 = w_in
            if generator.truncation_psi and generator.truncation_cutoff:
                psi = [generator.truncation_psi if j < generator.truncation_cutoff else 1.0 for j in range(len(mods))]
        self.styles = [self.buf(B, m.linear.weight.shape[0]) for m in mods]
        items = []
        for j, (m, st) in enumerate(zip(mods, self.styles)):
            lin = m.linear
            if generator is not None:
                items.append((self.w512, self.w512.stride(0), lin.weight, lin.bias, lin.w_lrmul * psi[j], lin.b_lrmul, LRELU, st))
            else:
                items.append((None, 0, lin.weight, lin.bias, lin.w_lrmul, lin.b_lrmul, LRELU, st))
        self.style_groups = self.fc_grouped(items, B)
        shapes = s.noise_shapes(B)
        sizes = [sh[0] * sh[2] * sh[3] for sh in shapes]
        self.noise_flat = self.buf(sum(sizes))
        self.noise_views = [t.view(sh) for t, sh in zip(self.noise_flat.split(sizes), shapes)]
        C0 = s.const_input.shape[1]
        pp = [self.buf(B * max(self._act_floats(s)))  for _ in range(2)]
        x = pp[0][:B * C0 * 16].view(B, C0, 4, 4)
        self.track(s.const_input, s.bias, s.noise_input1.weight)
        self.noise_ops = []
        d = self.add(L.OP_BIAS_NOISE_STYLE, L.BiasNoiseStyleArgs(
            x=L.dptr(s.const_input, "const_input"), x_batch_stride=0 if B > 1 else C0 * 16, bias=L.dptr(s.bias, "bias"),
            noise_w=L.dptr(s.noise_input1.weight, "noise_w"), noise=self.noise_views[0].data_ptr(), style=self.styles[0].data_ptr(),
            style_stride=self.styles[0].stride(0), y=x.data_ptr(), B=B, C=C0, HW=16))
        self.noise_ops.append(d)
        cur = 0
        for i, layer in enumerate(s.layers):
            for half, (conv, nmod) in enumerate(((layer.conv1, layer.noise1), (layer.conv2, layer.noise2))):
                Cout = conv.weight.shape[0]
                up = half == 0
                H = x.shape[2] * (2 if up else 1)
                y = pp[1 - cur][:B * Cout * H * H].view(B, Cout, H, H)
                k = 1 + 2 * i + half
                self.track(conv.bias, nmod.weight)
                last_conv = i == len(s.layers) - 1 and half == 1 and FUSE_TORGB and Cout <= 64 and s.to_rgb.weight.shape[0] == 3 and \
                    ops.conv3x3_route(B, x.shape[1], Cout, H, H, precision="f32")[0] == "wino" and ops.wino_ksplit(B, x.shape[1], Cout, H, H) == 1
                d = self.conv(x, conv.weight, Cout, bias=conv.bias, noise_w=nmod.weight, noise=self.noise_views[k],
                              style=self.styles[k], upsample=up, slope=LRELU, out=y, precision="f32" if last_conv else precision)
# ... 314 lines not shown
```

Measured before the change: 4020 frames/s.

## Add four-image Winograd region shape for 8x8 convs and adaptive FC row blocking

Adds a QUAD region shape to the Winograd f32 kernel that packs four batch images' 8x8 (or 4x4 upsampled) tiles into one 64-tile workgroup, so 8x8 layers that previously fell back to the direct conv can use Winograd with a k-split. Routing in ops/plan/autograd selects it for plain or bilinear-x2 8x8 convs when enough workgroups result, and adds a workspace query for the split partial sums. The wide FC kernel is templated on rows per block and uses 2 rows when 4 would underfill the CUs. The risks are a larger LDS footprint per block and the extra k-split reduction traffic.

After: 4044 frames/s, median of 6. About the same (+0.6%).

```diff
diff --git a/include/spk.h b/include/spk.h
--- a/include/spk.h
+++ b/include/spk.h
@@ -106,6 +106,8 @@
 int spk_conv2d_wino_up_supported(int B, int Cin, int Cout, int H, int W);
 int spk_conv2d_wino_ksplit(int want, int B, int Cin, int Cout, int H, int W);
 int64_t spk_conv2d_wino_workspace_bytes(int ksplit, int B, int Cin, int Cout, int H, int W);
+int spk_conv2d_wino_quad_ksplit(int want, int B, int Cin, int Cout, int H, int W);
+int64_t spk_conv2d_wino_quad_workspace_bytes(int ksplit, int B, int Cin, int Cout, int H, int W);
 int spk_conv2d_wino_fwd(const spk_conv2d_desc* desc, void* stream);
 
 typedef struct spk_wgrad_desc {
diff --git a/speak-hack_amd/_lib.py b/speak-hack_amd/_lib.py
--- a/speak-hack_amd/_lib.py
+++ b/speak-hack_amd/_lib.py
@@ -239,6 +239,8 @@
     "spk_conv2d_wino_up_supported": (C.c_int, [C.c_int] * 5),
     "spk_conv2d_wino_ksplit": (C.c_int, [C.c_int] * 6),
     "spk_conv2d_wino_workspace_bytes": (C.c_int64, [C.c_int] * 6),
+    "spk_conv2d_wino_quad_ksplit": (C.c_int, [C.c_int] * 6),
+    "spk_conv2d_wino_quad_workspace_bytes": (C.c_int64, [C.c_int] * 6),
     "spk_conv2d_wino_fwd": (C.c_int, [C.POINTER(Conv2dDesc), C.c_void_p]),
     "spk_conv2d_stats_slots": (C.c_int, [C.c_int] * 9),
     "spk_bn_finalize": (C.c_int, [C.c_void_p, C.c_int, C.c_int64, C.c_void_p, C.c_void_p, C.c_void_p, C.c_void_p, C.c_float,
diff --git a/speak-hack_amd/autograd.py b/speak-hack_amd/autograd.py
--- a/speak-hack_amd/autograd.py
+++ b/speak-hack_amd/autograd.py
@@ -130,7 +130,7 @@
         keep = _needs(ctx, grad_mode)
         a = torch.empty((B, Cout, H, W), device=x.device, dtype=torch.float32) if keep else None
         pw = getattr(weight, "_spk_gate_of", weight)
-        route = ops.conv3x3_route(B, Cin, Cout, H, W)
+        route = ops.conv3x3_route(B, Cin, Cout, H, W, quad=not keep)
         x2 = ops.upsample2x_bilinear(x) if upsample and route[0] == "wino" and keep else None
         y = ops.conv3x3(x if x2 is None else x2, packed.images(pw), Cout, route, upsample=upsample and x2 is None, bias=bias,
                         noise_w=noise_w, noise=noise, style=style, lrelu_slope=slope, out_pre=a, out_scale=w_scale)
diff --git a/speak-hack_amd/csrc/conv3x3_wino_f32.hip b/speak-hack_amd/csrc/conv3x3_wino_f32.hip
--- a/speak-hack_amd/csrc/conv3x3_wino_f32.hip
+++ b/speak-hack_amd/csrc/conv3x3_wino_f32.hip
@@ -11,8 +11,8 @@
 typedef __attribute__((address_space(3))) f32x2 __attribute__((aligned(4))) lds_f32x2u_t;
 
 constexpr int CO_T = 64, CI_T = 8, NTILE = 64, NT = 256;
-constexpr int WIDE = 0, SQUARE = 1;
-constexpr int region_w(int shape) { return shape == SQUARE ? 16 : 32; }
+constexpr int WIDE = 0, SQUARE = 1, QUAD = 2;
+constexpr int region_w(int shape) { return shape == QUAD ? 8 : shape == SQUARE ? 16 : 32; }
 constexpr int region_h(int shape) { return shape == SQUARE ? 16 : 8; }
 constexpr int RAW_PLANE = 352, RAW_WAVE = 2 * RAW_PLANE;
 constexpr int RAW_GATHERS = RAW_WAVE / 64;
@@ -28,6 +28,11 @@
 constexpr int UP_PLANE = 128, UP_GATHERS = 2 * UP_PLANE / 64;
 static_assert(18 * 6 <= UP_PLANE && 10 * 10 <= UP_PLANE && 2 * UP_PLANE <= RAW_WAVE, "geometry");
 constexpr int U_DMA = U_FLOATS * 4 / 1024 / 4;
+constexpr int raw_plane(int shape, bool up) { return shape == QUAD ? (up ? 144 : 400) : (up ? UP_PLANE : RAW_PLANE); }
+constexpr int raw_wave(int shape) { return shape == QUAD ? 832 : RAW_WAVE; }
+constexpr int lds_bytes(int shape) { return (LDS_FLOATS + 2 * 4 * (raw_wave(shape) - RAW_WAVE)) * 4; }
+static_assert(4 * 10 * 10 <= raw_plane(QUAD, false) && 4 * 6 * 6 <= raw_plane(QUAD, true) && 2 * raw_plane(QUAD, false) <= raw_wave(QUAD) &&
+              raw_wave(QUAD) % 64 == 0 && lds_bytes(QUAD) <= 160 * 1024 && lds_bytes(WIDE) == LDS_BYTES, "geometry");
 
 struct Args {
     const float* x;
@@ -150,16 +155,22 @@
 template <bool MOD, int SHAPE, bool RGB = false, bool UP = false>
 __global__ __launch_bounds__(NT) void wino_kernel(const Args p) {
     static_assert(!(UP && MOD), "the modulated conv keeps its x2 pass");
+    constexpr bool Q4 = SHAPE == QUAD;
+    static_assert(!(Q4 && (MOD || RGB)), "four-image regions: plain and bilinear x2 launches, raw partial sums");
     constexpr int RW = region_w(SHAPE), RH = region_h(SHAPE), TXN = RW / 2, TYN = RH / 2;
-    constexpr int RAW_W = UP ? RW / 2 + 2 : RW + 2, RAW_H = UP ? RH / 2 + 2 : RH + 2, RAW_USED = RAW_W * RAW_H;
-    constexpr int PLANE = UP ? UP_PLANE : RAW_PLANE, NG = UP ? UP_GATHERS : RAW_GATHERS;
+    constexpr int RAW_W = UP ? RW / 2 + 2 : RW + 2, RAW_H = UP ? RH / 2 + 2 : RH + 2;
+    constexpr int SUB = RAW_W * RAW_H, RAW_USED = Q4 ? 4 * SUB : SUB;
+    constexpr int PLANE = raw_plane(SHAPE, UP), NG = (2 * PLANE + 63) / 64;
+    constexpr int RAWW = raw_wave(SHAPE), RAWF = 4 * RAWW;
+    constexpr int PRM = RAW_OFF + 2 * RAWF, DEM = PRM + 4 * CO_T, RGBW = DEM + CO_T;
+    static_assert(NG == (Q4 ? (UP ? 5 : 13) : (UP ? UP_GATHERS : RAW_GATHERS)) && NG * 64 <= RAWW, "geometry");
     extern __shared__ __attribute__((aligned(16))) float smem[];
     const int tid = threadIdx.x, lane = tid & 63;
     const int wave = __builtin_amdgcn_readfirstlane(tid >> 6);
     const int half = lane >> 5, l32 = lane & 31;
     const int wm = wave >> 1, wn = wave & 1;
 
-    const int n_regions = p.regions_x * p.regions_y * p.B * p.ksplit;
+    const int n_regions = p.regions_x * p.regions_y * (Q4 ? p.B >> 2 : p.B) * p.ksplit;
     const int xcd = (int)blockIdx.x & 7, wk = (int)blockIdx.x >> 3, wpx = (int)gridDim.x >> 3;
     const int share_q = n_regions >> 3, share_r = n_regions & 7;
     const int reg_begin = xcd * share_q + min(xcd, share_r), reg_end = reg_begin + share_q + (xcd < share_r ? 1 : 0);
@@ -177,6 +188,7 @@
         const int t_ = reg / p.regions_x;
         b_ = t_ / p.regions_y;
         y0_ = (t_ - b_ * p.regions_y) * RH;
+        if constexpr (Q4) b_ *= 4;
         x0_ = rx_ * RW;
     };
     unsigned rel[NG], edge[NG];
@@ -184,8 +196,9 @@
     for (int k = 0; k < NG; ++k) {
         const int e = k * 64 + lane;
         const int j = e >= PLANE ? 1 : 0, q = e - j * PLANE;
-        const int r = q / RAW_W, c = q - r * RAW_W;
-        rel[k] = ((unsigned)(wave + 4 * j) * (unsigned)HWin + (unsigned)((r - 1) * Win + (c - 1))) * 4u;
+        const int img = Q4 ? q / SUB : 0, qi = q - img * SUB;
+        const int r = qi / RAW_W, c = qi - r * RAW_W;
+        rel[k] = (((unsigned)(wave + 4 * j) + (unsigned)img * (unsigned)p.Cx) * (unsigned)HWin + (unsigned)((r - 1) * Win + (c - 1))) * 4u;
         edge[k] = (r == 0 ? 1u : 0u) | (r == RAW_H - 1 ? 2u : 0u) | (c == 0 ? 4u : 0u) | (c == RAW_W - 1 ? 8u : 0u) | (q >= RAW_USED ? 16u : 0u);
     }
     auto set_voff = [&](unsigned (&vo)[NG], int b_, int y0_, int x0_) {
@@ -210,7 +223,7 @@
 
 #define WINO_DMA_RAW(vo_in_, chunk_, slot_, k_)                                                                         \
     {                                   \
-        const unsigned m0_ = (unsigned)((RAW_OFF + (slot_) * RAW_FLOATS + (k_) * 64) * 4) + raw_m0, vo_ = (vo_in_);     \
+        const unsigned m0_ = (unsigned)((RAW_OFF + (slot_) * RAWF + (k_) * 64) * 4) + raw_m0, vo_ = (vo_in_);           \
         const unsigned so_ = (unsigned)(chunk_) * chunk_bytes;                                                          \
         const __amdgpu_buffer_rsrc_t rs_ = rsrc;                                                                        \
         asm volatile("s_mov_b32 m0, %0\n\ts_nop 0\n\tbuffer_load_dword %1, %2, %3 offen lds" :: "s"(m0_), "v"(vo_), "s"(rs_), "s"(so_)); \
@@ -221,12 +234,13 @@
         const float* sb_ = wsrc + (size_t)(chunk_) * U_FLOATS + (wave * U_DMA + (k_)) * 256;                            \
         asm volatile("s_mov_b32 m0, %0\n\ts_nop 0\n\tglobal_load_lds_dwordx4 %1, %2" :: "s"(m0_), "v"(vo_), "s"(sb_));   \
     }
-    const unsigned raw_m0 = (unsigned)(wave * RAW_WAVE * 4), u_m0 = (unsigned)(wave * U_DMA * 1024), lane16 = (unsigned)lane * 16u;
+    const unsigned raw_m0 = (unsigned)(wave * RAWW * 4), u_m0 = (unsigned)(wave * U_DMA * 1024), lane16 = (unsigned)lane * 16u;
 
     int a_base = U_OFF + half * CO_T + wm * 32 + l32;
     int b_base = V_OFF + half * NTILE + wn * 32 + l32;
-    const int ty_l = lane / TXN, tx_l = lane % TXN;
-    int raw_rd = (RAW_OFF + wave * RAW_WAVE + 2 * ty_l * RAW_W + 2 * tx_l) >> 1;
+    const int lane_t = Q4 ? lane & 15 : lane, lane_sub = Q4 ? (lane >> 4) * SUB : 0;
+    const int ty_l = lane_t / TXN, tx_l = lane_t % TXN;
+    int raw_rd = (RAW_OFF + wave * RAWW + lane_sub + 2 * ty_l * RAW_W + 2 * tx_l) >> 1;
     int v_wr = V_OFF + wave * NTILE + lane;
     asm volatile("" : "+v"(a_base), "+v"(b_base), "+v"(raw_rd), "+v"(v_wr));
     int raw_u[2][2];
@@ -243,7 +257,7 @@
         for (int rs = 0; rs < 2; ++rs)
 #pragma unroll
             for (int j = 0; j < 2; ++j) {
-                raw_u[rs][j] = RAW_OFF + wave * RAW_WAVE + ty_l * RAW_W + tx_l + rs * RAW_FLOATS + j * PLANE;
+                raw_u[rs][j] = RAW_OFF + wave * RAWW + lane_sub + ty_l * RAW_W + tx_l + rs * RAWF + j * PLANE;
                 asm volatile("" : "+v"(raw_u[rs][j]));
             }
     }
@@ -256,8 +270,8 @@
     float d[2][16], tq[2][16], tv[2][16];
 #define WINO_T_READ(rs_, j_, r_)                                                                                        \
     {                                                                                                                   \
-        const f32x2 lo_ = *((const volatile lds_f32x2_t*)0 + (raw_rd + ((rs_) * RAW_FLOATS + (j_) * RAW_PLANE + (r_) * RAW_W) / 2)); \
-        const f32x2 hi_ = *((const volatile lds_f32x2_t*)0 + (raw_rd + ((rs_) * RAW_FLOATS + (j_) * RAW_PLANE + (r_) * RAW_W + 2) / 2)); \
+        const f32x2 lo_ = *((const volatile lds_f32x2_t*)0 + (raw_rd + ((rs_) * RAWF + (j_) * PLANE + (r_) * RAW_W) / 2)); \
+        const f32x2 hi_ = *((const volatile lds_f32x2_t*)0 + (raw_rd + ((rs_) * RAWF + (j_) * PLANE + (r_) * RAW_W + 2) / 2)); \
         d[j_][4 * (r_) + 0] = lo_.x; d[j_][4 * (r_) + 1] = lo_.y; d[j_][4 * (r_) + 2] = hi_.x; d[j_][4 * (r_) + 3] = hi_.y; \
     }
 #define WINO_T_ROWS(j_, c_)                                                                                             \
@@ -288,7 +302,7 @@
     *((volatile lds_f32_t*)0 + (v_wr + ((vs_) * V_FLOATS + ((xi_) * CI_T + 4 * (j_)) * NTILE))) = tv[j_][xi_];
 
     if constexpr (RGB) {
-        if (tid < 3 * CO_T) smem[RGBW_OFF + tid] = (tid & (CO_T - 1)) < p.Cout ? p.rgb_w[(tid >> 6) * p.Cout + (tid & (CO_T - 1))] : 0.f;
+        if (tid < 3 * CO_T) smem[RGBW + tid] = (tid & (CO_T - 1)) < p.Cout ? p.rgb_w[(tid >> 6) * p.Cout + (tid & (CO_T - 1))] : 0.f;
     }
     const int n = p.cps;
     int reg = reg_begin + wk;
@@ -374,7 +388,7 @@
     const bool f_lrelu = p.flags & SPK_EPI_LRELU, f_style = p.flags & SPK_EPI_STYLE, f_accum = p.flags & SPK_EPI_ACCUM;
     const float osc = p.out_scale_dev ? p.out_scale * *p.out_scale_dev : p.out_scale;
     const float slope_ = f_lrelu ? p.slope : 1.f, gain_ = f_lrelu ? p.act_gain : 1.f;
-    const int tile = wn * 32 + l32, oy = 2 * (tile / TXN), ox = 2 * (tile % TXN);
+    const int tile = wn * 32 + l32, tile_i = Q4 ? tile & 15 : tile, oy = 2 * (tile_i / TXN), ox = 2 * (tile_i % TXN);
     const int row_lane = wm * 32 + 4 * half;
     const int prm_which = tid & 3, prm_c = co0 + (tid >> 2);
     const bool prm_on = prm_c < p.Cout && (prm_which == 0 ? f_bias : (prm_which == 1 ? f_noise : f_style));
@@ -442,12 +456,12 @@
         }
 
         LAB_STAMP(2)
-        smem[PRM_OFF + tid] = prm;
-        if constexpr (MOD) { if (tid < CO_T) smem[DEM_OFF + tid] = dem; }
+        smem[PRM + tid] = prm;
+        if constexpr (MOD) { if (tid < CO_T) smem[DEM + tid] = dem; }
         lds_barrier();
         unsigned hw_ = (unsigned)HW;
         asm volatile("" : "+s"(hw_));
-        const size_t o0 = ((size_t)cur_b * p.Cy + (size_t)grp * p.Cout) * hw_ + pix + (size_t)(kb_cur / p.cps) * p.slice_floats;
+        const size_t o0 = ((size_t)(Q4 ? cur_b + (tile >> 4) : cur_b) * p.Cy + (size_t)grp * p.Cout) * hw_ + pix + (size_t)(kb_cur / p.cps) * p.slice_floats;
         LAB_STAMP(3)
 #define WINO_ACC(xi_, r_) ({ float v_; asm volatile("v_accvgpr_read_b32 %0, %1" : "=v"(v_) : "a"(acc[xi_][r_])); v_; })
         float rgb[3][4];
@@ -458,7 +472,7 @@
         static_for<0, 16>([&](auto r_c) {
             constexpr int r = decltype(r_c)::value;
             const int row = row_lane + (r & 3) + 8 * (r >> 2);
-            const float4 q_ = *reinterpret_cast<const float4*>(smem + PRM_OFF + 4 * row);
+            const float4 q_ = *reinterpret_cast<const float4*>(smem + PRM + 4 * row);
             float s0[4], s1[4];
 #pragma unroll
             for (int i = 0; i < 4; ++i) {
@@ -470,7 +484,7 @@
             top.x = (s0[0] + s0[1]) + s0[2]; top.y = (s1[0] + s1[1]) + s1[2];
             bot.x = (s0[1] - s0[2]) - s0[3]; bot.y = (s1[1] - s1[2]) - s1[3];
             float osc_r = osc;
-            if constexpr (MOD) osc_r = osc * smem[DEM_OFF + row];
+            if constexpr (MOD) osc_r = osc * smem[DEM + row];
             top.x = top.x * osc_r + q_.x; top.y = top.y * osc_r + q_.x; bot.x = bot.x * osc_r + q_.x; bot.y = bot.y * osc_r + q_.x;
             top.x += q_.y * nz0.x; top.y += q_.y * nz0.y; bot.x += q_.y * nz1.x; bot.y += q_.y * nz1.y;
             top.x = (top.x > 0.f ? top.x : top.x * slope_) * gain_; top.y = (top.y > 0.f ? top.y : top.y * slope_) * gain_;
@@ -480,7 +494,7 @@
                 top.x = top.x * q_.z + q_.w; top.y = top.y * q_.z + q_.w; bot.x = bot.x * q_.z + q_.w; bot.y = bot.y * q_.z + q_.w;
 #pragma unroll
                 for (int o = 0; o < 3; ++o) {
-                    const float w_ = smem[RGBW_OFF + o * CO_T + row];
+                    const float w_ = smem[RGBW + o * CO_T + row];
                     rgb[o][0] += w_ * top.x; rgb[o][1] += w_ * top.y; rgb[o][2] += w_ * bot.x; rgb[o][3] += w_ * bot.y;
                 }
                 if (p.y && co < p.Cout) {
@@ -615,10 +629,7 @@
     return 1;
 }
 
-int spk_conv2d_wino_ksplit(int want, int B, int Cin, int Cout, int H, int W) {
-    if (!wino_geometry_ok(B, Cin, Cout, H, W)) return -1;
-    const int shape = wino_shape(H, W), n_chunks = Cin / CI_T;
-    const long long pairs = (long long)B * (H / region_h(shape)) * (W / region_w(shape)) * spk::ceil_div(Cout, CO_T);
+static int wino_pick_ksplit(int want, long long pairs, int n_chunks) {
     auto ok = [&](int ks) { return ks >= 1 && n_chunks % (2 * ks) == 0 && n_chunks / ks >= 4; };
     if (want > 0) {
         int ks = want;
@@ -628,6 +639,26 @@
     int ks = 1;
     while (pairs * ks < 192 && ok(2 * ks)) ks *= 2;
     return ks;
+}
+
+int spk_conv2d_wino_ksplit(int want, int B, int Cin, int Cout, int H, int W) {
+    if (!wino_geometry_ok(B, Cin, Cout, H, W)) return -1;
+    const int shape = wino_shape(H, W);
+    return wino_pick_ksplit(want, (long long)B * (H / region_h(shape)) * (W / region_w(shape)) * spk::ceil_div(Cout, CO_T), Cin / CI_T);
+}
+
+static int wino_quad_ok(int B, int Cin, int Cout, int H, int W) {
+    return B > 0 && Cout > 0 && H == 8 && W == 8 && B % 4 == 0 && Cin >= 8 * CI_T && Cin % (2 * CI_T) == 0 && (long long)B * Cin * H * W * 4 < (1ll << 31);
+}
+
+int spk_conv2d_wino_quad_ksplit(int want, int B, int Cin, int Cout, int H, int W) {
+    if (!wino_quad_ok(B, Cin, Cout, H, W)) return -1;
+    return wino_pick_ksplit(want, (long long)(B / 4) * spk::ceil_div(Cout, CO_T), Cin / CI_T);
+}
+
+int64_t spk_conv2d_wino_quad_workspace_bytes(int ksplit, int B, int Cin, int Cout, int H, int W) {
+    const int ks = spk_conv2d_wino_quad_ksplit(ksplit, B, Cin, Cout, H, W);
+    return ks < 2 ? -1 : (int64_t)ks * B * Cout * H * W * 4;
 }
 
 int64_t spk_conv2d_wino_workspace_bytes(int ksplit, int B, int Cin, int Cout, int H, int W) {
@@ -653,6 +684,8 @@
     SPK_REQUIRE(!(d->flags & ~allowed) && !d->stats && !d->accum_half,
                 "conv2d winograd: plain, bilinear x2 or batch-scaled input; epilogue flags bias, noise, lrelu, style, accum, torgb");
     const bool mod = d->flags & SPK_CONV_IN_BATCH_SCALE, rgb = d->flags & SPK_EPI_TORGB;
+    const bool quad = wino_shape(d->H, d->W) < 0 && wino_quad_ok(d->B, d->Cin, d->Cout, d->H, d->W);
+    SPK_REQUIRE(!quad || (G == 1 && !mod && !rgb), "conv2d winograd: an 8x8 output runs plain or bilinear x2, ungrouped, without toRGB");
     SPK_REQUIRE(d->y || rgb, "conv2d winograd: null pointer");
     if (rgb)
         SPK_REQUIRE(d->rgb_w && d->rgb_y && d->rgb_channels == 3 && d->Cout <= CO_T && !mod && !d->y_pre && !(d->flags & SPK_EPI_ACCUM) &&
@@ -661,20 +694,24 @@
     SPK_REQUIRE(!mod || d->in_scale, "conv2d winograd: IN_BATCH_SCALE without in_scale[B,Cin]");
     SPK_REQUIRE(!d->out_scale_bc || mod, "conv2d winograd: out_scale_bc (demodulation) goes with SPK_CONV_IN_BATCH_SCALE");
     if (up)
-        SPK_REQUIRE(d->H == 2 * d->Hin && d->W == 2 * d->Win && spk_conv2d_wino_up_supported(d->B, d->Cin, d->Cout, d->H, d->W),
+        SPK_REQUIRE(d->H == 2 * d->Hin && d->W == 2 * d->Win && (quad || spk_conv2d_wino_up_supported(d->B, d->Cin, d->Cout, d->H, d->W)),
                     "conv2d winograd: SPK_CONV_UPSAMPLE2X needs an output of twice the input size, %dx%d -> %dx%d", d->Hin, d->Win, d->H, d->W);
     else
         SPK_REQUIRE(d->H == d->Hin && d->W == d->Win, "conv2d winograd: output size must equal the input size");
-    SPK_REQUIRE(wino_geometry_ok(d->B, d->Cin, d->Cout, d->H, d->W) && (long long)d->B * Cx * d->Hin * d->Win * 4 < (1ll << 31),
-                "conv2d winograd: %dx%d is not a whole number of 32 x 8 or 16 x 16 regions (or the input exceeds 2 GB)", d->H, d->W);
+    SPK_REQUIRE((quad || wino_geometry_ok(d->B, d->Cin, d->Cout, d->H, d->W)) && (long long)d->B * Cx * d->Hin * d->Win * 4 < (1ll << 31),
+                "conv2d winograd: %dx%d is not a whole number of 32 x 8 or 16 x 16 regions, nor 8x8 with B %% 4 == 0 and Cin >= 64 "
+                "(or the input exceeds 2 GB)", d->H, d->W);
     SPK_REQUIRE(!(d->flags & SPK_EPI_BIAS) || d->bias, "conv2d winograd: SPK_EPI_BIAS without bias");
     SPK_REQUIRE(!(d->flags & SPK_EPI_NOISE) || (d->noise && d->noise_w), "conv2d winograd: SPK_EPI_NOISE without noise");
     SPK_REQUIRE(!(d->flags & SPK_EPI_STYLE) || d->style, "conv2d winograd: SPK_EPI_STYLE without style");
     const auto aligned16 = [](const void* q) { return (reinterpret_cast<uintptr_t>(q) & 15) == 0; };
     SPK_REQUIRE(aligned16(d->w_packed) && aligned16(d->y) && aligned16(d->y_pre) && aligned16(d->noise) && (reinterpret_cast<uintptr_t>(d->x) & 3) == 0,
                 "conv2d winograd: tensors must be 16-byte aligned");
-    const int shape = wino_shape(d->H, d->W);
-    const int ks = spk_conv2d_wino_ksplit(d->ksplit, d->B, d->Cin, Cy, d->H, d->W);
+    const int shape = quad ? QUAD : wino_shape(d->H, d->W);
+    const int ks = quad ? spk_conv2d_wino_quad_ksplit(d->ksplit, d->B, d->Cin, Cy, d->H, d->W)
+                        : spk_conv2d_wino_ksplit(d->ksplit, d->B, d->Cin, Cy, d->H, d->W);
+    SPK_REQUIRE(!quad || ks >= 2, "conv2d winograd: an 8x8 output is always sliced (raw partial sums, the finisher applies the epilogue): "
+                "ksplit %d resolves to %d -- pass 0 or >= 2", d->ksplit, ks);
     const size_t out_floats = (size_t)d->B * Cy * d->H * d->W;
     if (ks > 1)
         SPK_REQUIRE(d->workspace && aligned16(d->workspace) && d->workspace_bytes >= (int64_t)ks * (int64_t)out_floats * 4,
@@ -705,14 +742,15 @@
     if (up)
         kern = rgb ? (shape == SQUARE ? &wino_kernel<false, SQUARE, true, true> : &wino_kernel<false, WIDE, true, true>)
                    : (shape == SQUARE ? &wino_kernel<false, SQUARE, false, true> : &wino_kernel<false, WIDE, false, true>);
-    static bool raised[10] = {false, false, false, false, false, false, false, false, false, false};
-    const int which = (mod ? 2 : rgb ? 4 : 0) + (shape == SQUARE ? 1 : 0) + (up ? (rgb ? 4 : 6) : 0);
+    if (quad) kern = up ? &wino_kernel<false, QUAD, false, true> : &wino_kernel<false, QUAD>;
+    static bool raised[12] = {false, false, false, false, false, false, false, false, false, false, false, false};
+    const int which = quad ? (up ? 11 : 10) : (mod ? 2 : rgb ? 4 : 0) + (shape == SQUARE ? 1 : 0) + (up ? (rgb ? 4 : 6) : 0);
     if (!raised[which]) {
         hipError_t e = hipFuncSetAttribute(reinterpret_cast<const void*>(kern), hipFuncAttributeMaxDynamicSharedMemorySize, 160 * 1024);
         if (e != hipSuccess) return spk::fail(SPK_ELAUNCH, "hipFuncSetAttribute(LDS): %s", hipGetErrorString(e));
         raised[which] = true;
     }
-    const long long n_items = (long long)a.regions_x * a.regions_y * d->B * ks;
+    const long long n_items = (long long)a.regions_x * a.regions_y * (quad ? d->B / 4 : d->B) * ks;
     SPK_REQUIRE(n_items < (1ll << 31), "conv2d winograd: grid too large");
     const int co_tiles = G * spk::ceil_div(d->Cout, CO_T);
     static int n_cu = 0;
@@ -728,7 +766,7 @@
     gx = lab_mult == 0 ? (n_items + 7) / 8 * 8 : gx * lab_mult;
     gx = std::min(gx, (n_items + 7) / 8 * 8);
     dim3 grid((unsigned)gx, (unsigned)co_tiles);
-    hipLaunchKernelGGL(kern, grid, dim3(NT), LDS_BYTES, (hipStream_t)stream, a);
+    hipLaunchKernelGGL(kern, grid, dim3(NT), lds_bytes(shape), (hipStream_t)stream, a);
     int rc = spk::check_launch("wino_kernel");
     if (rc != SPK_OK || ks == 1) return rc;
     spkconv::ConvArgs f = {};
diff --git a/speak-hack_amd/csrc/fc.hip b/speak-hack_amd/csrc/fc.hip
--- a/speak-hack_amd/csrc/fc.hip
+++ b/speak-hack_amd/csrc/fc.hip
@@ -129,23 +129,24 @@
     }
 }
 
-__global__ __launch_bounds__(256) void fc_wide4_kernel(const float* __restrict__ x, long long x_stride, const float* __restrict__ w,
+template <int R>
+__global__ __launch_bounds__(256) void fc_wide_rows_kernel(const float* __restrict__ x, long long x_stride, const float* __restrict__ w,
                                                       const float* __restrict__ bias, float* __restrict__ out, long long out_stride,
                                                       int B, int I, int O, float wmul, float bmul, float slope) {
-    __shared__ float red[4][4][FC_BT];
+    __shared__ float red[4][R][FC_BT];
     const int tid = threadIdx.x, lane = tid & 63, wave = tid >> 6;
-    const int o0 = blockIdx.x * 4;
+    const int o0 = blockIdx.x * R;
     const int U = I >> 10;
-    float4 wv[4][FC_WIDE_U];
-#pragma unroll
-    for (int r = 0; r < 4; ++r)
+    float4 wv[R][FC_WIDE_U];
+#pragma unroll
+    for (int r = 0; r < R; ++r)
 #pragma unroll
         for (int u = 0; u < FC_WIDE_U; ++u)
             wv[r][u] = *reinterpret_cast<const float4*>(w + (size_t)(o0 + r) * I + tid * 4 + min(u, U - 1) * 1024);
     for (int b0 = 0; b0 < B; b0 += FC_BT) {
-        float acc[4][FC_BT];
-#pragma unroll
-        for (int r = 0; r < 4; ++r)
+        float acc[R][FC_BT];
+#pragma unroll
+        for (int r = 0; r < R; ++r)
 #pragma unroll
             for (int b = 0; b < FC_BT; ++b) acc[r][b] = 0.f;
 #pragma unroll
@@ -156,14 +157,14 @@
                 for (int b = 0; b < FC_BT; ++b)
                     xv[b] = *reinterpret_cast<const float4*>(x + (size_t)min(b0 + b, B - 1) * x_stride + tid * 4 + u * 1024);
 #pragma unroll
-                for (int r = 0; r < 4; ++r)
+                for (int r = 0; r < R; ++r)
 #pragma unroll
                     for (int b = 0; b < FC_BT; ++b)
                         acc[r][b] += wv[r][u].x * xv[b].x + wv[r][u].y * xv[b].y + wv[r][u].z * xv[b].z + wv[r][u].w * xv[b].w;
             }
         }
 #pragma unroll
-        for (int r = 0; r < 4; ++r)
+        for (int r = 0; r < R; ++r)
 #pragma unroll
             for (int b = 0; b < FC_BT; ++b) {
 #pragma unroll
@@ -172,12 +173,12 @@
         __syncthreads();
         if (lane == 0) {
 #pragma unroll
-            for (int r = 0; r < 4; ++r)
+            for (int r = 0; r < R; ++r)
 #pragma unroll
                 for (int b = 0; b < FC_BT; ++b) red[wave][r][b] = acc[r][b];
         }
         __syncthreads();
-        if (tid < 4 * FC_BT) {
+        if (tid < R * FC_BT) {
             const int r = tid / FC_BT, b = tid % FC_BT;
             if (b0 + b < B) {
                 float v = (red[0][r][b] + red[1][r][b]) + (red[2][r][b] + red[3][r][b]);
@@ -248,9 +249,20 @@
     SPK_REQUIRE(x_stride >= I && out_stride >= O, "fc: row stride smaller than row");
     const bool vec = (I % 4 == 0) && (x_stride % 4 == 0) && ((uintptr_t)x % 16 == 0) && ((uintptr_t)w % 16 == 0);
     if (vec && I >= 2048 && I % 1024 == 0 && I <= 1024 * FC_WIDE_U && O % 4 == 0) {
-        hipLaunchKernelGGL(fc_wide4_kernel, dim3((unsigned)(O / 4)), dim3(256), 0, (hipStream_t)stream, x, (long long)x_stride, w, bias, out,
-                           (long long)out_stride, B, I, O, wmul, bmul, slope);
-        return spk::check_launch("fc_wide4_kernel");
+        static int n_cu = 0;
+        if (n_cu == 0) {
+            int dev = 0;
+            hipDeviceProp_t prop;
+            if (hipGetDevice(&dev) != hipSuccess || hipGetDeviceProperties(&prop, dev) != hipSuccess) return spk::fail(SPK_ELAUNCH, "fc: no device properties");
+            n_cu = prop.multiProcessorCount > 0 ? prop.multiProcessorCount : 256;
+        }
+        if (O / 4 < n_cu)
+            hipLaunchKernelGGL(fc_wide_rows_kernel<2>, dim3((unsigned)(O / 2)), dim3(256), 0, (hipStream_t)stream, x, (long long)x_stride, w, bias,
+                               out, (long long)out_stride, B, I, O, wmul, bmul, slope);
+        else
+            hipLaunchKernelGGL(fc_wide_rows_kernel<4>, dim3((unsigned)(O / 4)), dim3(256), 0, (hipStream_t)stream, x, (long long)x_stride, w, bias,
+                               out, (long long)out_stride, B, I, O, wmul, bmul, slope);
+        return spk::check_launch("fc_wide_rows_kernel");
     }
     if (vec && I >= 2048) {
         hipLaunchKernelGGL(fc_wide_kernel, dim3((unsigned)O), dim3(256), 0, (hipStream_t)stream, x, (long long)x_stride, w, bias, out,
diff --git a/speak-hack_amd/ops.py b/speak-hack_amd/ops.py
--- a/speak-hack_amd/ops.py
+++ b/speak-hack_amd/ops.py
@@ -77,6 +77,8 @@
             raise L.SpkError(f"conv2d: config {config} cannot host k={k} s={stride} shape {(B, Cin, Cout, H, W)}")
     elif kind == L.CONV_WINOGRAD:
         ws_bytes = L.lib().spk_conv2d_wino_workspace_bytes(int(ksplit), B, Cin, G * Cout, H, W)
+        if ws_bytes < 0 and G == 1:
+            ws_bytes = L.lib().spk_conv2d_wino_quad_workspace_bytes(int(ksplit), B, Cin, Cout, H, W)
     elif kind == L.CONV_DGRAD_S2:
         ws_bytes = L.lib().spk_conv2d_dgrad_s2_workspace_bytes(B, Cin, Cout, Hs, Ws, H, W, G)
     else:
@@ -307,6 +309,7 @@
 CONV3X3_ALGO = os.environ.get("SPK_CONV3X3_ALGO", "auto")
 WINO_MIN_WORKGROUPS = 192
 WINO_FUSE_X2 = os.environ.get("SPK_WINO_FUSE_X2", "1") != "0"
+WINO_8X8 = os.environ.get("SPK_WINO_8X8", "1") != "0"
 
 
 @contextlib.contextmanager
@@ -321,8 +324,12 @@
         CONV3X3_ALGO = prev
 
 
-def use_wino(B, Cin, Cout, H, W, groups=1) -> bool:
-    if CONV3X3_ALGO != "auto" or not wino_supported(B, Cin, Cout, H, W):
+def use_wino(B, Cin, Cout, H, W, groups=1, quad=False) -> bool:
+    if CONV3X3_ALGO != "auto":
+        return False
+    if quad and WINO_8X8 and groups == 1 and wino_quad_supported(B, Cin, Cout, H, W):
+        return (B // 4) * ((Cout + 63) // 64) * wino_ksplit(B, Cin, Cout, H, W) >= WINO_MIN_WORKGROUPS
+    if not wino_supported(B, Cin, Cout, H, W):
         return False
     rw, rh = (32, 8) if (W % 32 == 0 and H % 8 == 0) else (16, 16)
     tiles = groups * ((Cout + 63) // 64)
@@ -330,7 +337,12 @@
 
 
 def wino_ksplit(B, Cin, Cout, H, W, want=0) -> int:
-    return int(L.lib().spk_conv2d_wino_ksplit(int(want), B, Cin, Cout, H, W))
+    ks = int(L.lib().spk_conv2d_wino_ksplit(int(want), B, Cin, Cout, H, W))
+    return ks if ks > 0 else int(L.lib().spk_conv2d_wino_quad_ksplit(int(want), B, Cin, Cout, H, W))
+
+
+def wino_quad_supported(B, Cin, Cout, H, W) -> bool:
+    return L.lib().spk_conv2d_wino_quad_ksplit(0, B, Cin, Cout, H, W) >= 2
 
 
 def wino_supported(B, Cin, Cout, H, W) -> bool:
@@ -338,7 +350,11 @@
 
 
 def wino_fuse_x2(B, Cin, Cout, H, W, up_fir=False, modulated=False) -> bool:
-    return bool(WINO_FUSE_X2 and not up_fir and not modulated and L.lib().spk_conv2d_wino_up_supported(B, Cin, Cout, H, W))
+    if up_fir or modulated:
+        return False
+    if wino_quad_supported(B, Cin, Cout, H, W):
+        return True
+    return bool(WINO_FUSE_X2 and L.lib().spk_conv2d_wino_up_supported(B, Cin, Cout, H, W))
 
 
 def pack_conv_weight_wino(weight: torch.Tensor, out=None, transpose_flip=False) -> torch.Tensor:
@@ -431,9 +447,11 @@
     return config + 4 if modulated and config < 4 else config
 
 
-def conv3x3_route(B, Cin, Cout, H, W, *, precision=None, groups=1, modulated=False, up_w=None, wino_ok=True):
+def conv3x3_route(B, Cin, Cout, H, W, *, precision=None, groups=1, modulated=False, up_w=None, wino_ok=True, quad=False):
     if _bf16x3_route(TRAIN_CONV_PRECISION if precision is None else precision, B, Cin, Cout, H, W):
         return "bf16x3", -1
+    if wino_ok and quad and not modulated and groups == 1 and H == W == 8 and use_wino(B, Cin, Cout, H, W, quad=True):
+        return "wino", -1
     if wino_ok and (up_w is None or up_w % 4 == 0) and use_wino(B, Cin, Cout, H, W, groups):
         return "wino", -1
     return "direct", _modulated_config(conv2d_pick_config(3, 1, B, Cin, Cout, H, W), modulated)
diff --git a/speak-hack_amd/plan.py b/speak-hack_amd/plan.py
--- a/speak-hack_amd/plan.py
+++ b/speak-hack_amd/plan.py
@@ -49,7 +49,7 @@
         B, Cin, Hs, Ws = x.shape
         H, W = (2 * Hs, 2 * Ws) if upsample else (Hs, Ws)
         kind, cfg = ops.conv3x3_route(B, Cin, Cout, H, W, precision=precision, modulated=batch_scale is not None,
-                                      up_w=Ws if upsample else None)
+                                      up_w=Ws if upsample else None, quad=batch_scale is None and not up_fir)
         up_op = None
         if kind == "wino" and upsample and ops.wino_fuse_x2(B, Cin, Cout, H, W, up_fir, modulated=batch_scale is not None):
             pass
```
